# hongfz16/Garment4D

Measured on AMD Instinct MI355X. Metric: point-cloud frames/s (FPS+ball_query+SA-MLP+LBS), B=8 N=8192, higher is better.
Workload: dtype f32

## Files before the change

garment4d_amd/_lib.py:

```python
import ctypes
import os
import re
import sys

_HERE = os.path.dirname(os.path.abspath(__file__))
LIB_PATH = os.environ.get("G4D_LIB_PATH") or os.path.join(_HERE, "lib", "libg4d_hip.so")
HEADER_PATH = os.path.join(os.path.dirname(_HERE), "include", "g4d.h")

RENDER_LIB_PATH = os.path.join(_HERE, "lib", "libg4d_render.so")
RENDER_HEADER_PATH = os.path.join(os.path.dirname(_HERE), "include", "g4d_render.h")
SCAN_LIB_PATH = os.path.join(_HERE, "lib", "libg4d_scan.so")
SCAN_HEADER_PATH = os.path.join(os.path.dirname(_HERE), "include", "g4d_scan.h")
FIT_LIB_PATH = os.path.join(_HERE, "lib", "libg4d_fit.so")
FIT_HEADER_PATH = os.path.join(os.path.dirname(_HERE), "include", "g4d_fit.h")
SMPL_LIB_PATH = os.path.join(_HERE, "lib", "libg4d_smpl.so")
SMPL_HEADER_PATH = os.path.join(os.path.dirname(_HERE), "include", "g4d_smpl.h")
SKIN_LIB_PATH = os.path.join(_HERE, "lib", "libg4d_skin.so")
SKIN_HEADER_PATH = os.path.join(os.path.dirname(_HERE), "include", "g4d_skin.h")
DEPTH_LIB_PATH = os.path.join(_HERE, "lib", "libg4d_depth.so")
DEPTH_HEADER_PATH = os.path.join(os.path.dirname(_HERE), "include", "g4d_depth.h")

SETS_HEADER_PATH = os.path.join(os.path.dirname(_HERE), "include", "g4d_sets.h")

_lib = None
_header = None
_more = {}


class G4DError(RuntimeError):
    pass


_SCALARS = {"int": ctypes.c_int, "float": ctypes.c_float, "long long": ctypes.c_longlong, "size_t": ctypes.c_size_t, "unsigned": ctypes.c_uint}


def _ctype(decl, where, named=True):
    base, star, rest = decl.partition("*")
    words = [w for w in base.split() if w != "const"]
    if named and not star:
        words.pop()
    base = " ".join(words)
    if star:
        return ctypes.c_char_p if base == "char" and "*" not in rest else ctypes.c_void_p
    if base == "g4d_stream_t":
        return ctypes.c_void_p
    if base not in _SCALARS:
        raise G4DError(f"include/g4d.h: {where}: no ctypes type known for `{' '.join(decl.split())}`")
    return _SCALARS[base]


def parse_header(text):
    text = re.sub(r"/\*.*?\*/", " ", text, flags=re.S)
    consts = {n: int(v, 0) for n, v in re.findall(r"^[ \t]*#[ \t]*define[ \t]+(G4D_\w+)[ \t]+(-?(?:0[xX][0-9a-fA-F]+|\d+))[ \t]*$", text, flags=re.M)}
    text = re.sub(r"^[ \t]*#.*$", "", text, flags=re.M)
    for body in re.findall(r"\benum\s+\w+\s*\{(.*?)\}", text, flags=re.S):
        consts.update((n, int(v, 0)) for n, v in re.findall(r"(G4D_\w+)\s*=\s*(-?\w+)", body))
    fields = []
    struct = re.search(r"\bstruct\s+g4d_mlp_args\s*\{(.*?)\}", text, flags=re.S)
    for decl in filter(str.strip, struct.group(1).split(";") if struct else ()):
        first, *more = decl.split(",")
        base = first.partition("*")[0] if "*" in first else first.rsplit(None, 1)[0]
        for piece in [first] + [base + " " + p for p in more]:
            fields.append((re.findall(r"\w+", piece)[-1], _ctype(piece, "g4d_mlp_args")))
    protos = {}
    for stmt in re.split(r"[;{}]", text):
        if "(" not in stmt:
            continue
        m = re.fullmatch(r"\s*([\w\s*]+?)\b(g4d_\w+)\s*\(([^()]*)\)\s*", stmt)
        if not m:
            raise G4DError(f"include/g4d.h: cannot read `{' '.join(stmt.split())}` as a prototype")
        ret, name, params = m.groups()
        params = [] if params.strip() in ("void", "") else params.split(",")
        protos[name] = (_ctype(ret, name, named=False), [_ctype(p, name) for p in params])
    return protos, fields, consts


_MLP_FAMILY_LABELS = {"G4D_MLP_STACK_F32": "g4d_mlp_stack_f32", "G4D_MLP_STACK_BF16": "g4d_mlp_stack_bf16", "G4D_MLP_WAVE_F32": "g4d_mlp_wave_f32",
                      "G4D_MLP_CHAIN_F32": "g4d_mlp_chain_f32", "G4D_MLP_CHAIN_BF16": "g4d_mlp_chain_bf16", "G4D_MLP_CHAIN_BF16X3": "g4d_mlp_chain_bf16x3"}


def _bind_header():
    global _header
    try:
        with open(HEADER_PATH) as f:
            protos, fields, consts = parse_header(f.read())
    except OSError as e:
        raise G4DError(f"{HEADER_PATH} cannot be read ({e.strerror}): the ctypes binding is derived from it. There is no fallback table.")

    class MlpArgs(ctypes.Structure):
        _fields_ = fields

        def __init__(self, **kw):
            super().__init__(size=ctypes.sizeof(MlpArgs), version=consts["G4D_MLP_ARGS_VERSION"], tap_layer=-1, **kw)

    globals().update(
        PROTOTYPES=protos, SIGNATURES={n: a for n, (r, a) in protos.items()}, RESTYPES={n: r for n, (r, a) in protos.items() if r is not ctypes.c_int},
        CONSTANTS=consts, MlpArgs=MlpArgs, _MLP_FAMILY_NAMES={consts[k]: v for k, v in _MLP_FAMILY_LABELS.items()},
        **{k[4:]: v for k, v in consts.items() if k.startswith("G4D_MLP_")})
    _header = HEADER_PATH


def __getattr__(name):
    if _header is None and not name.startswith("__"):
        _bind_header()
        if name in globals():
            return globals()[name]
    raise AttributeError(f"module {__name__!r} has no attribute {name!r}")


def lib():
    global _lib
    if _lib is None:
        if not os.path.exists(LIB_PATH):
            raise G4DError(
                f"{LIB_PATH} not found: the HIP extension is not built. Run `python -c 'import "
                f"__graft_entry__ as g; g.build()'` (or `make -C garment4d_amd/csrc`). There is no fallback path.")
        if _header is None:
            _bind_header()
        import torch
        L = ctypes.CDLL(LIB_PATH)
        for name, (restype, argtypes) in PROTOTYPES.items():
            fn = getattr(L, name)
            fn.argtypes = argtypes
            fn.restype = restype
        _lib = L
    return _lib


def load_pair(header_path, lib_path):
    if lib_path not in _more:
        lib()
        if not os.path.exists(lib_path):
            raise G4DError(f"{lib_path} not found: the HIP extension is not built. Run `python -c 'import __graft_entry__ as g; g.build()'` "
                           f"(or `make -C garment4d_amd/csrc`). There is no fallback path.")
        try:
            with open(header_path) as f:
                protos, _, consts = parse_header(f.read())
        except OSError as e:
            raise G4DError(f"{header_path} cannot be read ({e.strerror}): the ctypes binding is derived from it. There is no fallback table.")
        L = ctypes.CDLL(lib_path)
        for name, (restype, argtypes) in protos.items():
            fn = getattr(L, name)
            fn.argtypes = argtypes
            fn.restype = restype
        _more[lib_path] = (L, protos, consts)
    return _more[lib_path]


def render_lib():
    return load_pair(RENDER_HEADER_PATH, RENDER_LIB_PATH)


def scan_lib():
    return load_pair(SCAN_HEADER_PATH, SCAN_LIB_PATH)


def fit_lib():
    return load_pair(FIT_HEADER_PATH, FIT_LIB_PATH)


def smpl_lib():
    return load_pair(SMPL_HEADER_PATH, SMPL_LIB_PATH)


def skin_lib():
    return load_pair(SKIN_HEADER_PATH, SKIN_LIB_PATH)


def depth_lib():
    return load_pair(DEPTH_HEADER_PATH, DEPTH_LIB_PATH)


def sets_lib():
    return load_pair(SETS_HEADER_PATH, LIB_PATH)


def _entry(name):
    L = lib()
    if name not in PROTOTYPES:
        for M, protos, _ in _more.values():
            if name in protos:
                return getattr(M, name)
    return getattr(L, name)


_TRACE = os.environ.get("G4D_TRACE_CALLS", "0") != "0"
_TIMED = None
_UNTIMED = ("g4d_tuning_set", "g4d_tuning_set_thread", "g4d_launch_group_begin")


class timed_calls:

    def __enter__(self):
        global _TIMED
        self._rec = []
        _TIMED = self._rec
        return self

    def __exit__(self, *exc):
        global _TIMED
        _TIMED = None
        return False

    def results(self):
        import torch
        torch.cuda.synchronize()
        return [(name, ints, e0.elapsed_time(e1) * 1e3) for name, ints, e0, e1 in self._rec]


def call(name, *args):
    L = lib()
    fn = _entry(name)
    timed = _TIMED is not None and args and name not in _UNTIMED
    if _TRACE or timed:
        label, shown = name, tuple(a for a in args if isinstance(a, int) and not isinstance(a, bool) and abs(a) < (1 << 31))
        if name == "g4d_mlp_run":
            blk = args[1].contents if hasattr(args[1], "contents") else MlpArgs.from_address(args[1])
            label = _MLP_FAMILY_NAMES[args[0]] if blk.unknown_grid is None else "g4d_mlp_chain_cells_bf16"
            shown = (blk.mode, blk.rows, blk.K0, blk.ldx, blk.N, blk.P, blk.S, blk.C, blk.use_xyz, blk.n, blk.m, blk.C2, blk.C1, blk.nlayers, blk.pool)
            if _TRACE:
                print("g4d call g4d_mlp_run ->", label, *shown, file=sys.stderr)
        if _TRACE:
            print("g4d call", name, *[a for a in args if isinstance(a, (int, float)) and abs(a) < (1 << 31)], file=sys.stderr)
    if timed:
        import torch
        e0, e1 = torch.cuda.Event(enable_timing=True), torch.cuda.Event(enable_timing=True)
        e0.record()
        rc = fn(*args)
        e1.record()
        _TIMED.append((label, shown, e0, e1))
    else:
        rc = fn(*args)
    if rc != 0:
        raise G4DError(f"{name} failed with status {rc}: {L.g4d_last_error().decode(errors='replace')}")
    return rc


def host_array(ctype, values):
    return ctypes.cast((ctype * len(values))(*values), ctypes.c_void_p)


def workspace(nbytes, device):
    import torch
    return torch.empty(max(int(nbytes), 16), dtype=torch.uint8, device=device)


def ver(t):
    try:
        return t._version
    except RuntimeError:
        return None


def stream_ptr():
    import torch
    return torch.cuda.current_stream().cuda_stream
```

garment4d_amd/csrc/ball_grid.hip:

```cpp
#include <cstdlib>

#include "g4d_common.h"
#include "../../include/g4d_sets.h"
#include "ball_grid_build.h"

namespace g4d {

__global__ void __launch_bounds__(kBuildThreads) ball_grid_build_kernel(int n, int cmax, int budget, float cell_req, const float *__restrict__ xyz_all,
                                                                       unsigned char *__restrict__ ws_all, size_t ws_stride) {
    ball_grid_build_body(n, cmax, budget, cell_req, xyz_all, ws_all, ws_stride, blockIdx.x);
}

struct BgArgs {
    float radius2[4];
    int nsample[4];
    int *idx[4];
};

__device__ __forceinline__ int query_cell(float v, float lo, float inv_c, int g) {
    const float u = floorf((v - lo) * inv_c);
    return (int)fminf(fmaxf(u, -2.f), (float)(g + 1));
}

template <int NS, int FM, bool SET>
__global__ void __launch_bounds__(256) ball_grid_query_kernel(int n, int m, int qpw, const BgArgs a, const float *__restrict__ new_xyz_all,
                                                             const float *__restrict__ xyz_all, const unsigned char *__restrict__ ws_all,
                                                             size_t ws_stride, int cmax) {
    __shared__ int lst[4][NS][kCap];
    const int t = threadIdx.x, lane = t & 63;
    const int wave = __builtin_amdgcn_readfirstlane(t >> 6);
    const int b = blockIdx.y;
    const unsigned char *ws = ws_all + (size_t)b * ws_stride;
    const GridHdr *hdr = reinterpret_cast<const GridHdr *>(ws);
    const int *cellstart = reinterpret_cast<const int *>(ws + kGridHdrBytes);
    const float4 *sorted = reinterpret_cast<const float4 *>(ws + kGridHdrBytes + ((((size_t)cmax + 1) * 4 + 63) & ~(size_t)63));
    const float *xyz = xyz_all + (size_t)b * n * 3;
    const float lox = hdr->lox, loy = hdr->loy, loz = hdr->loz, inv_c = hdr->inv_c;
    const int gx = hdr->gx, gy = hdr->gy, gz = hdr->gz;
    const int ry = lane % 3 - 1, rz = (lane / 3) % 3 - 1;

    for (int qi = 0; qi < qpw; ++qi) {
        const int q = (blockIdx.x * 4 + wave) * qpw + qi;
        if (q >= m) break;
        const float *qp = new_xyz_all + ((size_t)b * m + q) * 3;
        const float qx = qp[0], qy = qp[1], qz = qp[2];
        const int cx = query_cell(qx, lox, inv_c, gx), cy = query_cell(qy, loy, inv_c, gy), cz = query_cell(qz, loz, inv_c, gz);
        const int x0 = max(cx - 1, 0), x1 = min(cx + 1, gx - 1);
        const int yy = cy + ry, zz = cz + rz;
        int s = 0, e = 0;
        if (lane < 9 && x0 <= x1 && yy >= 0 && yy < gy && zz >= 0 && zz < gz) {
            const int row = (zz * gy + yy) * gx;
            s = cellstart[row + x0];
            e = cellstart[row + x1 + 1];
        }
        int cum[10], off[9];
        cum[0] = 0;
#pragma unroll
        for (int r = 0; r < 9; ++r) {
            const int rs = __builtin_amdgcn_readlane(s, r), re = __builtin_amdgcn_readlane(e, r);
            off[r] = rs - cum[r];
            cum[r + 1] = cum[r] + (re - rs);
        }
        const int total = cum[9];
        int h[NS];
#pragma unroll
        for (int sc = 0; sc < NS; ++sc) h[sc] = 0;

        for (int j0 = 0; j0 < total; j0 += 4 * 64) {
            bool all_dense = true;
#pragma unroll
            for (int sc = 0; sc < NS; ++sc) all_dense &= h[sc] > kCap;
            if (all_dense) break;
            float4 p[4];
            bool valid[4];
#pragma unroll
            for (int u = 0; u < 4; ++u) {
                const int j = j0 + u * 64 + lane;
                valid[u] = j < total;
                int o = off[0];
#pragma unroll
                for (int r = 1; r < 9; ++r) o = (j >= cum[r]) ? off[r] : o;
                p[u] = sorted[valid[u] ? j + o : 0];
            }
#pragma unroll
            for (int u = 0; u < 4; ++u) {
                if (j0 + u * 64 >= total) break;
                const float d2 = dist2<FM>(qx - p[u].x, qy - p[u].y, qz - p[u].z);
#pragma unroll
                for (int sc = 0; sc < NS; ++sc) {
                    const bool hit = valid[u] && d2 < a.radius2[sc];
                    const unsigned long long mask = __builtin_amdgcn_ballot_w64(hit);
                    if (mask != 0ull) {
                        const int slot = h[sc] + (int)__builtin_amdgcn_mbcnt_hi((unsigned)(mask >> 32), __builtin_amdgcn_mbcnt_lo((unsigned)mask, 0u));
                        if (hit && slot < kCap) lst[wave][sc][slot] = __float_as_int(p[u].w);
                        h[sc] += __builtin_popcountll(mask);
                    }
                }
            }
        }

#pragma unroll
        for (int sc = 0; sc < NS; ++sc) {
            const int ns = a.nsample[sc];
            int *out = a.idx[sc] + ((size_t)b * m + q) * ns;
            const int hs = h[sc];
            if (hs == 0) {
                for (int l = lane; l < ns; l += 64) out[l] = 0;
            } else if (hs <= kCap) {
                int *L = lst[wave][sc];
                int hacc = hs;
                if (hs > ns) {
                    int v[kCapRegs];
#pragma unroll
                    for (int e = 0; e < kCapRegs; ++e) v[e] = (e * 64 + lane < hs) ? L[e * 64 + lane] : 0x7fffffff;
                    const int ne = (hs + 63) >> 6;
                    int lo = 0, hi = n;
                    while (lo < hi) {
                        const int mid = (lo + hi) >> 1;
                        int c = 0;
#pragma unroll
                        for (int e = 0; e < kCapRegs; ++e)
                            if (e < ne) c += __builtin_popcountll(__builtin_amdgcn_ballot_w64(v[e] < mid));
                        if (c >= ns) hi = mid; else lo = mid + 1;
                    }
                    int w = 0;
#pragma unroll
                    for (int e = 0; e < kCapRegs; ++e)
                        if (e < ne) {
                            const bool keep = v[e] < lo;
                            const unsigned long long mask = __builtin_amdgcn_ballot_w64(keep);
                            const int slot = w + (int)__builtin_amdgcn_mbcnt_hi((unsigned)(mask >> 32), __builtin_amdgcn_mbcnt_lo((unsigned)mask, 0u));
                            if (keep) L[slot] = v[e];
                            w += __builtin_popcountll(mask);
                        }
                    hacc = w;
                }
                if constexpr (SET) {
                    const int first = L[0];
                    for (int l = lane; l < ns; l += 64) out[l] = l < hacc ? L[l] : first;
                    continue;
                }
                int first = 0;
                for (int i0 = 0; i0 < hacc; i0 += 64) {
                    const int i = i0 + lane;
                    const int v = i < hacc ? L[i] : 0x7fffffff;
                    int rank = 0;
#pragma unroll 4
                    for (int j = 0; j < hacc; ++j) rank += (L[j] < v) ? 1 : 0;
                    if (i < hacc && rank < ns) out[rank] = v;
                    const unsigned long long z = __builtin_amdgcn_ballot_w64(i < hacc && rank == 0);
                    if (z != 0ull) first = __builtin_amdgcn_readlane(v, __builtin_ctzll(z));
                }
                for (int l = hacc + lane; l < ns; l += 64) out[l] = first;
            } else {
                const float r2 = a.radius2[sc];
                int cnt = 0, first = 0;
                for (int base = 0; base < n && cnt < ns; base += 64) {
                    const int k = base + lane;
                    const int kc = min(k, n - 1);
                    const float d2 = dist2<FM>(qx - xyz[kc * 3 + 0], qy - xyz[kc * 3 + 1], qz - xyz[kc * 3 + 2]);
                    const bool hit = k < n && d2 < r2;
                    const unsigned long long mask = __builtin_amdgcn_ballot_w64(hit);
                    if (mask != 0ull) {
                        if (cnt == 0) first = base + __builtin_ctzll(mask);
                        const int slot = cnt + (int)__builtin_amdgcn_mbcnt_hi((unsigned)(mask >> 32), __builtin_amdgcn_mbcnt_lo((unsigned)mask, 0u));
                        if (hit && slot < ns) out[slot] = k;
                        cnt += __builtin_popcountll(mask);
                    }
                }
                for (int l = cnt + lane; l < ns; l += 64) out[l] = first;
            }
        }
    }
}

__device__ __forceinline__ void nn3_insert_lex(float d, int k, float &b1, float &b2, float &b3, int &i1, int &i2, int &i3) {
    const bool lt1 = d < b1 || (d == b1 && k < i1), lt2 = d < b2 || (d == b2 && k < i2), lt3 = d < b3 || (d == b3 && k < i3);
    const float nb3 = lt2 ? b2 : (lt3 ? d : b3);
    const int ni3 = lt2 ? i2 : (lt3 ? k : i3);
    const float nb2 = lt1 ? b1 : (lt2 ? d : b2);
    const int ni2 = lt1 ? i1 : (lt2 ? k : i2);
    b1 = lt1 ? d : b1; i1 = lt1 ? k : i1;
    b2 = nb2; i2 = ni2; b3 = nb3; i3 = ni3;
}

template <int FM, bool STAGE>
__global__ void __launch_bounds__(256) three_nn_grid_kernel(int n, int m, const float *__restrict__ unknown_all,
                                                           const unsigned char *__restrict__ ws_all, size_t ws_stride, int cmax,
                                                           float *__restrict__ dist2_all, int *__restrict__ idx_all) {
    extern __shared__ __attribute__((aligned(16))) unsigned char nn_smem[];
    const int b = blockIdx.y;
    const int p = blockIdx.x * 256 + threadIdx.x;
    const unsigned char *ws = ws_all + (size_t)b * ws_stride;
    const GridHdr h = *reinterpret_cast<const GridHdr *>(ws);
    const int *cellstart = reinterpret_cast<const int *>(ws + kGridHdrBytes);
    const float4 *rec = reinterpret_cast<const float4 *>(ws + kGridHdrBytes + ((((size_t)cmax + 1) * 4 + 63) & ~(size_t)63));
    if constexpr (STAGE) {
        float4 *srec = reinterpret_cast<float4 *>(nn_smem);
        int *scell = reinterpret_cast<int *>(nn_smem + (size_t)m * 16);
        for (int k = threadIdx.x; k < m; k += 256) srec[k] = rec[k];
        for (int k = threadIdx.x; k <= h.ncells; k += 256) scell[k] = cellstart[k];
        __syncthreads();
        rec = srec;
        cellstart = scell;
    }
    const float *u = unknown_all + ((size_t)b * n + min(p, n - 1)) * 3;
    const float ux = u[0], uy = u[1], uz = u[2];
    const float INF = __builtin_inff();
    float b1 = INF, b2 = INF, b3 = INF;
    int i1 = 0, i2 = 0, i3 = 0;
    auto visit = [&](int k0, int k1) {
        int k = k0;
        for (; k + 1 < k1; k += 2) {
            const float4 r0 = rec[k], r1 = rec[k + 1];
            const float d0 = dist2<FM>(ux - r0.x, uy - r0.y, uz - r0.z);
            const float d1 = dist2<FM>(ux - r1.x, uy - r1.y, uz - r1.z);
            nn3_insert_lex(d0, __float_as_int(r0.w), b1, b2, b3, i1, i2, i3);
            nn3_insert_lex(d1, __float_as_int(r1.w), b1, b2, b3, i1, i2, i3);
        }
        if (k < k1) {
            const float4 r0 = rec[k];
            nn3_insert_lex(dist2<FM>(ux - r0.x, uy - r0.y, uz - r0.z), __float_as_int(r0.w), b1, b2, b3, i1, i2, i3);
        }
    };
    const float fx = (ux - h.lox) * h.inv_c, fy = (uy - h.loy) * h.inv_c, fz = (uz - h.loz) * h.inv_c;
    bool pending = true;
    const bool local = fx > -1.f && fx < (float)h.gx + 1.f && fy > -1.f && fy < (float)h.gy + 1.f && fz > -1.f && fz < (float)h.gz + 1.f;
    if (local) {
        const int cx = (int)floorf(fx), cy = (int)floorf(fy), cz = (int)floorf(fz);
        const float edge = h.inv_c > 0.f ? 1.0f / h.inv_c : INF;
        {
            const int x0 = max(cx - 1, 0), x1 = min(cx + 1, h.gx - 1);
            int rs[9], re[9];
#pragma unroll
            for (int q = 0; q < 9; ++q) {
                const int y = cy + (q % 3) - 1, z = cz + (q / 3) - 1;
                const bool ok = x0 <= x1 && y >= 0 && y < h.gy && z >= 0 && z < h.gz;
                const int row = ok ? (z * h.gy + y) * h.gx : 0;
                rs[q] = ok ? cellstart[row + x0] : 0;
                re[q] = ok ? cellstart[row + x1 + 1] : 0;
            }
#pragma unroll
            for (int q = 0; q < 9; ++q) visit(rs[q], re[q]);
            const float reach = edge * 0.99f;
            pending = !(b3 < reach * reach);
        }
        if (pending) {
            b1 = b2 = b3 = INF; i1 = i2 = i3 = 0;
            const int x0 = max(cx - 2, 0), x1 = min(cx + 2, h.gx - 1);
            if (x0 <= x1) {
                for (int dz = -2; dz <= 2; ++dz) {
                    const int z = cz + dz;
                    if (z < 0 || z >= h.gz) continue;
                    for (int dy = -2; dy <= 2; ++dy) {
                        const int y = cy + dy;
                        if (y < 0 || y >= h.gy) continue;
                        const int row = (z * h.gy + y) * h.gx;
                        visit(cellstart[row + x0], cellstart[row + x1 + 1]);
                    }
                }
            }
            const float reach = 2.f * edge * 0.99f;
            pending = !(b3 < reach * reach);
        }
    }
    if (pending) {
        b1 = b2 = b3 = INF; i1 = i2 = i3 = 0;
        visit(0, m);
    }
    if (p < n) {
        float *d2 = dist2_all + ((size_t)b * n + p) * 3;
        int *ix = idx_all + ((size_t)b * n + p) * 3;
        d2[0] = b1; d2[1] = b2; d2[2] = b3;
        ix[0] = i1; ix[1] = i2; ix[2] = i3;
    }
}

void grid_sorted_layout(int n, size_t *offset_bytes, size_t *stride_bytes) {
    *offset_bytes = kGridHdrBytes + ((((size_t)grid_cmax(n) + 1) * 4 + 63) & ~(size_t)63);
    *stride_bytes = grid_cloud_bytes(n);
}

int grid_build(int b, int n, float rmax, const float *xyz, void *ws, hipStream_t st, int budget) {
    const int cmax = grid_cmax(n);
    if (budget <= 0 || budget > cmax) budget = cmax;
    const size_t lds = ((size_t)cmax + 1) * 4 + 16 * 8 * 4;
    static unsigned long long attr = 0;
    if (const int rc = ensure_dynamic_lds(reinterpret_cast<const void *>(ball_grid_build_kernel), 160 * 1024 - 1024, attr, "g4d_ball_grid_build_f32"))
        return rc;
    hipLaunchKernelGGL(ball_grid_build_kernel, dim3(b), dim3(kBuildThreads), lds, st, n, cmax, budget, rmax > 0.f ? rmax * kCellSlack : 0.f, xyz,
                       reinterpret_cast<unsigned char *>(ws), grid_cloud_bytes(n));
    return check_launch("g4d_ball_grid_build_f32");
}

size_t grid_bytes_per_cloud(int n) { return grid_cloud_bytes(n); }
size_t grid_records_offset(int n) { return kGridHdrBytes + ((((size_t)grid_cmax(n) + 1) * 4 + 63) & ~(size_t)63); }

template <int NS, int FM, bool SET>
static void grid_query_launch(dim3 grid, hipStream_t st, int n, int m, int qpw, const BgArgs &a, const float *new_xyz, const float *xyz,
                              const void *ws) {
    hipLaunchKernelGGL((ball_grid_query_kernel<NS, FM, SET>), grid, dim3(256), 0, st, n, m, qpw, a, new_xyz, xyz,
                       reinterpret_cast<const unsigned char *>(ws), grid_cloud_bytes(n), grid_cmax(n));
}

template <bool SET>
static int grid_query(int b, int n, int m, int nscales, const float *radii, const int *nsamples, const float *new_xyz, const float *xyz,
                      int *const *idx, const void *ws, hipStream_t st) {
    BgArgs a = {};
    for (int s = 0; s < nscales; ++s) {
        a.radius2[s] = radii[s] * radii[s];
        a.nsample[s] = nsamples[s];
        a.idx[s] = idx[s];
    }
    const long long queries = (long long)b * m;
    int qpw = 1;
    while (qpw < 8 && queries / (qpw * 2) >= 32768) qpw <<= 1;
    static const int qpw_env = env_int("G4D_BG_QPW", 0);
    if (qpw_env > 0) qpw = qpw_env;
    dim3 grid((unsigned)((m + 4 * qpw - 1) / (4 * qpw)), (unsigned)b);
    G4D_WITH_FM(distance_contraction(), switch (nscales) {
        case 1: grid_query_launch<1, FM, SET>(grid, st, n, m, qpw, a, new_xyz, xyz, ws); break;
        case 2: grid_query_launch<2, FM, SET>(grid, st, n, m, qpw, a, new_xyz, xyz, ws); break;
        case 3: grid_query_launch<3, FM, SET>(grid, st, n, m, qpw, a, new_xyz, xyz, ws); break;
        default: grid_query_launch<4, FM, SET>(grid, st, n, m, qpw, a, new_xyz, xyz, ws); break;
    })
    return check_launch(SET ? "g4d_ball_grid_query_set_f32" : "g4d_ball_grid_query_f32");
}

template <bool SET>
static int grid_query_entry(const char *name, int b, int n, int m, int nscales, const float *radii, const int *nsamples, const float *new_xyz,
                            const float *xyz, int *const *idx, const void *grid, float grid_rmax, g4d_stream_t stream) {
    G4D_REQUIRE(b >= 0 && n >= 0 && m >= 0 && nscales >= 1 && nscales <= 4 && b <= 65535, "%s: bad sizes", name);
    G4D_REQUIRE(radii && nsamples && idx, "%s: null pointer", name);
    if (b == 0 || m == 0) return G4D_OK;
    hipStream_t st = reinterpret_cast<hipStream_t>(stream);
    for (int s = 0; s < nscales; ++s) {
        G4D_REQUIRE(nsamples[s] > 0 && idx[s], "%s: bad scale %d", name, s);
        G4D_REQUIRE(radii[s] <= grid_rmax, "%s: radius %g exceeds the radius the grid was built for (%g)", name, radii[s], grid_rmax);
        if (n == 0) {
            hipError_t e = hipMemsetAsync(idx[s], 0, sizeof(int) * (size_t)b * m * nsamples[s], st);
            if (e != hipSuccess) return (int)e;
        }
    }
    if (n == 0) return G4D_OK;
    G4D_REQUIRE(new_xyz && xyz && grid, "%s: null pointer", name);
    return grid_query<SET>(b, n, m, nscales, radii, nsamples, new_xyz, xyz, idx, grid, st);
}

}

extern "C" size_t g4d_ball_grid_bytes(int b, int n) {
    if (b <= 0 || n <= 0) return 0;
    return (size_t)b * g4d::grid_cloud_bytes(n);
}

extern "C" int g4d_ball_grid_build_f32(int b, int n, float rmax, const float *xyz, void *grid, g4d_stream_t stream) {
    using namespace g4d;
    G4D_REQUIRE(b >= 0 && n >= 0 && b <= 65535, "g4d_ball_grid_build_f32: bad sizes (b=%d n=%d)", b, n);
    if (b == 0 || n == 0) return G4D_OK;
    G4D_REQUIRE(xyz && grid, "g4d_ball_grid_build_f32: null pointer");
    G4D_REQUIRE(rmax > 0.f && rmax < __builtin_inff(), "g4d_ball_grid_build_f32: rmax must be a positive finite radius");
    return grid_build(b, n, rmax, xyz, grid, reinterpret_cast<hipStream_t>(stream));
}

extern "C" int g4d_ball_grid_query_f32(int b, int n, int m, int nscales, const float *radii, const int *nsamples, const float *new_xyz,
                                       const float *xyz, int *const *idx, const void *grid, float grid_rmax, g4d_stream_t stream) {
    return g4d::grid_query_entry<false>("g4d_ball_grid_query_f32", b, n, m, nscales, radii, nsamples, new_xyz, xyz, idx, grid, grid_rmax, stream);
}

extern "C" int g4d_ball_grid_query_set_f32(int b, int n, int m, int nscales, const float *radii, const int *nsamples, const float *new_xyz,
                                           const float *xyz, int *const *idx, const void *grid, float grid_rmax, g4d_stream_t stream) {
    return g4d::grid_query_entry<true>("g4d_ball_grid_query_set_f32", b, n, m, nscales, radii, nsamples, new_xyz, xyz, idx, grid, grid_rmax, stream);
}

extern "C" int g4d_ball_query_grid_f32(int b, int n, int m, int nscales, const float *radii, const int *nsamples, const float *new_xyz,
                                       const float *xyz, int *const *idx, void *grid, g4d_stream_t stream) {
    using namespace g4d;
    G4D_REQUIRE(nscales >= 1 && nscales <= 4 && radii, "g4d_ball_query_grid_f32: bad scales");
    float rmax = radii[0];
    for (int s = 1; s < nscales; ++s) rmax = radii[s] > rmax ? radii[s] : rmax;
    if (b > 0 && n > 0 && m > 0) {
        const int rc = g4d_ball_grid_build_f32(b, n, rmax, xyz, grid, stream);
        if (rc != G4D_OK) return rc;
    }
    return g4d_ball_grid_query_f32(b, n, m, nscales, radii, nsamples, new_xyz, xyz, idx, grid, rmax, stream);
}

extern "C" int g4d_three_nn_grid_f32(int b, int n, int m, const float *unknown, const float *known, float *dist2, int *idx, void *grid,
                                     g4d_stream_t stream) {
    using namespace g4d;
    G4D_REQUIRE(b >= 0 && n >= 0 && m >= 0 && b <= 65535, "g4d_three_nn_grid_f32: bad sizes (b=%d n=%d m=%d)", b, n, m);
    if ((long long)b * n == 0) return G4D_OK;
    G4D_REQUIRE(unknown && dist2 && idx, "g4d_three_nn_grid_f32: null pointer");
    if (m == 0) return g4d_three_nn_f32(b, n, m, unknown, known, dist2, idx, stream);
    G4D_REQUIRE(known && grid, "g4d_three_nn_grid_f32: null pointer (grid scratch = g4d_ball_grid_bytes(b, m))");
    hipStream_t st = reinterpret_cast<hipStream_t>(stream);
    static const int per_cell = [] { const char *e = getenv("G4D_NN_PER_CELL"); return e && atoi(e) > 0 ? atoi(e) : 1; }();
    if (const int rc = grid_build(b, m, 0.f, known, grid, st, m / per_cell > 8 ? m / per_cell : 8)) return rc;
    dim3 g((unsigned)((n + 255) / 256), (unsigned)b);
    const unsigned char *wsb = reinterpret_cast<const unsigned char *>(grid);
    if (m <= 2048) {
        const size_t lds = (size_t)m * 16 + ((size_t)grid_cmax(m) + 1) * 4;
        G4D_WITH_FM(distance_contraction(), hipLaunchKernelGGL((three_nn_grid_kernel<FM, true>), g, dim3(256), lds, st, n, m, unknown, wsb,
                                                              grid_cloud_bytes(m), grid_cmax(m), dist2, idx))
    } else {
        G4D_WITH_FM(distance_contraction(), hipLaunchKernelGGL((three_nn_grid_kernel<FM, false>), g, dim3(256), 0, st, n, m, unknown, wsb,
                                                              grid_cloud_bytes(m), grid_cmax(m), dist2, idx))
    }
    return check_launch("g4d_three_nn_grid_f32");
}
```

garment4d_amd/csrc/fps.hip:

```cpp
#include "g4d_common.h"

namespace g4d {

template <int U>
__device__ __host__ constexpr int brev_small(int v) {
    int r = 0;
    for (int bit = 1, rb = U >> 1; bit < U; bit <<= 1, rb >>= 1)
        if (v & bit) r |= rb;
    return r;
}

struct FpsCand {
    float val;
    unsigned rank;
    int k;
    int pad;
};

__device__ __forceinline__ void wave_argmax(float best, int k, int bs, int log2bs, float &wval, int &wk, unsigned &wrank) {
    wval = wave_max_f32(best);
    const unsigned long long hit = __builtin_amdgcn_ballot_w64(best == wval);
    int lane;
    if (__builtin_popcountll(hit) == 1) {
        lane = __builtin_ctzll(hit);
        wk = __builtin_amdgcn_readlane(k, lane);
        wrank = fps_rank(wk, bs, log2bs);
    } else {
        const unsigned r = (best == wval) ? fps_rank(k, bs, log2bs) : 0xffffffffu;
        wrank = wave_min_u32(r);
        lane = __builtin_ctzll(__builtin_amdgcn_ballot_w64(r == wrank));
        wk = __builtin_amdgcn_readlane(k, lane);
    }
}

template <int W, int U, int Q, int FM>
__global__ void __launch_bounds__(64 * W) fps_reg_kernel(int n, int m, int bs, int log2bs, const float *__restrict__ xyz_all,
                                                        float *__restrict__ temp_all, int *__restrict__ idx_all, float *__restrict__ nx_all) {
    constexpr int T = 64 * W, P = U * Q;
    extern __shared__ __attribute__((aligned(16))) unsigned char smem_raw[];
    float *sx = reinterpret_cast<float *>(smem_raw + 2 * 16 * 16);
    float *sy = sx + n;
    float *sz = sy + n;
    int *spick = reinterpret_cast<int *>(sz + n);

    const int t = threadIdx.x;
    const float *xyz = xyz_all + (size_t)blockIdx.x * n * 3;
    float *temp = temp_all + (size_t)blockIdx.x * n;
    int *idx = idx_all + (size_t)blockIdx.x * m;
    float *nx = nx_all ? nx_all + (size_t)blockIdx.x * m * 3 : nullptr;

    float px[P], py[P], pz[P], md[P];
#pragma unroll
    for (int i = 0; i < P; ++i) {
        const int k = t + brev_small<U>(i / Q) * T + (i % Q) * bs;
        const bool ok = k < n;
        px[i] = ok ? xyz[k * 3 + 0] : 0.f;
        py[i] = ok ? xyz[k * 3 + 1] : 0.f;
        pz[i] = ok ? xyz[k * 3 + 2] : 0.f;
        md[i] = ok ? (temp_all ? temp[k] : 1e10f) : -2.f;
        if (ok) { sx[k] = px[i]; sy[k] = py[i]; sz[k] = pz[i]; }
    }
    if (t == 0) spick[0] = 0;
    __syncthreads();

    float x1 = sx[0], y1 = sy[0], z1 = sz[0];
    const int wave = t >> 6;
    for (int j = 1; j < m; ++j) {
        float best = -1.f;
        int bslot = 0;
#pragma unroll
        for (int i = 0; i < P; ++i) {
            const float dx = px[i] - x1, dy = py[i] - y1, dz = pz[i] - z1;
            const float d = dist2<FM>(dx, dy, dz);
            const float d2 = bare_min_f32(d, md[i]);
            md[i] = d2;
            const bool gt = d2 > best;
            bslot = gt ? i : bslot;
            best = gt ? d2 : best;
        }
        int k;
        if constexpr (P == 1) k = t;
        else k = t + brev_small<U>(bslot / Q) * T + (bslot % Q) * bs;
        float wval; int wk; unsigned wrank;
        wave_argmax(best, k, bs, log2bs, wval, wk, wrank);
        int old;
        if constexpr (W == 1) {
            old = wk;
        } else {
            unsigned long long *buf = reinterpret_cast<unsigned long long *>(smem_raw) + (j & 1) * 16;
            if ((t & 63) == 0)
                buf[wave] = ((unsigned long long)__float_as_uint(fmaxf(wval, 0.f)) << 32) | (unsigned)(~wrank);
            __syncthreads();
            const unsigned long long key = row_max_u64<W>(buf[t & (W - 1)]);
            const unsigned rank = ~(unsigned)__builtin_amdgcn_readlane((int)(unsigned)key, W - 1);
            const unsigned c = log2bs ? (__builtin_bitreverse32(rank >> 16) >> (32 - log2bs)) : 0u;
            old = (int)(((rank & 0xffffu) << log2bs) | c);
        }
        x1 = sx[old]; y1 = sy[old]; z1 = sz[old];
        if (t == 0) spick[j] = old;
    }
    if constexpr (W > 1) __syncthreads();
    for (int j = t; j < m; j += T) {
        const int k = spick[j];
        idx[j] = k;
        if (nx) { nx[j * 3 + 0] = sx[k]; nx[j * 3 + 1] = sy[k]; nx[j * 3 + 2] = sz[k]; }
    }
    if (temp_all) {
#pragma unroll
        for (int i = 0; i < P; ++i) {
            const int k = t + brev_small<U>(i / Q) * T + (i % Q) * bs;
            if (k < n) temp[k] = md[i];
        }
    }
}

template <int UA, int UB, int FM>
__global__ void __launch_bounds__(256) fps_reg_pair_kernel(int m2, const float *__restrict__ xyz_all, int *__restrict__ idx1_all,
                                                          float *__restrict__ nx1_all, int *__restrict__ idx2_all, float *__restrict__ nx2_all) {
    constexpr int T = 256, W = 4, nA = T * UA, bsA = nA, m1 = 64 * UB, bsB = m1;
    constexpr int log2bsA = UA == 1 ? 8 : (UA == 2 ? 9 : 10), log2bsB = UB == 1 ? 6 : (UB == 2 ? 7 : (UB == 4 ? 8 : 9));
    extern __shared__ __attribute__((aligned(16))) unsigned char smem_raw[];
    float *sx = reinterpret_cast<float *>(smem_raw + 2 * 16 * 16);
    float *sy = sx + nA;
    float *sz = sy + nA;
    int *spick = reinterpret_cast<int *>(sz + nA);
    float *bx = reinterpret_cast<float *>(spick + m1);
    float *by = bx + m1;
    float *bz = by + m1;
    int *spick2 = reinterpret_cast<int *>(bz + m1);
    const int t = threadIdx.x;
    const float *xyz = xyz_all + (size_t)blockIdx.x * nA * 3;

    {
        float px[UA], py[UA], pz[UA], md[UA];
#pragma unroll
        for (int i = 0; i < UA; ++i) {
            const int k = t + brev_small<UA>(i) * T;
            px[i] = xyz[k * 3 + 0]; py[i] = xyz[k * 3 + 1]; pz[i] = xyz[k * 3 + 2];
            md[i] = 1e10f;
            sx[k] = px[i]; sy[k] = py[i]; sz[k] = pz[i];
        }
        if (t == 0) spick[0] = 0;
        __syncthreads();
        float x1 = sx[0], y1 = sy[0], z1 = sz[0];
        const int wave = t >> 6;
        for (int j = 1; j < m1; ++j) {
            float best = -1.f;
            int bslot = 0;
#pragma unroll
            for (int i = 0; i < UA; ++i) {
                const float dx = px[i] - x1, dy = py[i] - y1, dz = pz[i] - z1;
                const float d = dist2<FM>(dx, dy, dz);
                const float d2 = bare_min_f32(d, md[i]);
                md[i] = d2;
                const bool gt = d2 > best;
                bslot = gt ? i : bslot;
                best = gt ? d2 : best;
            }
            const int k = UA == 1 ? t : t + brev_small<UA>(bslot) * T;
            float wval; int wk; unsigned wrank;
            wave_argmax(best, k, bsA, log2bsA, wval, wk, wrank);
            unsigned long long *buf = reinterpret_cast<unsigned long long *>(smem_raw) + (j & 1) * 16;
            if ((t & 63) == 0) buf[wave] = ((unsigned long long)__float_as_uint(fmaxf(wval, 0.f)) << 32) | (unsigned)(~wrank);
            __syncthreads();
            const unsigned long long key = row_max_u64<W>(buf[t & (W - 1)]);
            const unsigned rank = ~(unsigned)__builtin_amdgcn_readlane((int)(unsigned)key, W - 1);
            const unsigned c = __builtin_bitreverse32(rank >> 16) >> (32 - log2bsA);
            const int old = (int)(((rank & 0xffffu) << log2bsA) | c);
            x1 = sx[old]; y1 = sy[old]; z1 = sz[old];
            if (t == 0) spick[j] = old;
        }
        __syncthreads();
        int *idx = idx1_all + (size_t)blockIdx.x * m1;
        float *nx = nx1_all + (size_t)blockIdx.x * m1 * 3;
        for (int j = t; j < m1; j += T) {
            const int k = spick[j];
            idx[j] = k;
            const float x = sx[k], y = sy[k], z = sz[k];
            nx[j * 3 + 0] = x; nx[j * 3 + 1] = y; nx[j * 3 + 2] = z;
            bx[j] = x; by[j] = y; bz[j] = z;
        }
        __syncthreads();
    }
    if (t >= 64) return;
    {
        float px[UB], py[UB], pz[UB], md[UB];
#pragma unroll
        for (int i = 0; i < UB; ++i) {
            const int k = t + brev_small<UB>(i) * 64;
            px[i] = bx[k]; py[i] = by[k]; pz[i] = bz[k];
            md[i] = 1e10f;
        }
        if (t == 0) spick2[0] = 0;
        float x1 = bx[0], y1 = by[0], z1 = bz[0];
        for (int j = 1; j < m2; ++j) {
            float best = -1.f;
            int bslot = 0;
#pragma unroll
            for (int i = 0; i < UB; ++i) {
                const float dx = px[i] - x1, dy = py[i] - y1, dz = pz[i] - z1;
                const float d = dist2<FM>(dx, dy, dz);
                const float d2 = bare_min_f32(d, md[i]);
                md[i] = d2;
                const bool gt = d2 > best;
                bslot = gt ? i : bslot;
                best = gt ? d2 : best;
            }
            const int k = UB == 1 ? t : t + brev_small<UB>(bslot) * 64;
            float wval; int wk; unsigned wrank;
            wave_argmax(best, k, bsB, log2bsB, wval, wk, wrank);
            const int old = wk;
            x1 = bx[old]; y1 = by[old]; z1 = bz[old];
            if (t == 0) spick2[j] = old;
        }
        __builtin_amdgcn_fence(__ATOMIC_RELEASE, "wavefront");
        __builtin_amdgcn_wave_barrier();
        __builtin_amdgcn_fence(__ATOMIC_ACQUIRE, "wavefront");
        int *idx = idx2_all + (size_t)blockIdx.x * m2;
        float *nx = nx2_all + (size_t)blockIdx.x * m2 * 3;
        for (int j = t; j < m2; j += 64) {
            const int k = spick2[j];
            idx[j] = k;
            nx[j * 3 + 0] = bx[k]; nx[j * 3 + 1] = by[k]; nx[j * 3 + 2] = bz[k];
        }
    }
}

template <int FM>
__global__ void __launch_bounds__(1024) fps_generic_kernel(int n, int m, int bs, int log2bs, const float *__restrict__ xyz_all,
                                                          float *__restrict__ temp_all, int *__restrict__ idx_all, float *__restrict__ nx_all) {
    constexpr int W = 16;
    __shared__ FpsCand slots[2][W];
    const int t = threadIdx.x;
    const float *xyz = xyz_all + (size_t)blockIdx.x * n * 3;
    float *temp = temp_all + (size_t)blockIdx.x * n;
    int *idx = idx_all + (size_t)blockIdx.x * m;
    float *nx = nx_all ? nx_all + (size_t)blockIdx.x * m * 3 : nullptr;
    if (t == 0) idx[0] = 0;
    int old = 0;
    const int wave = t >> 6;
    for (int j = 1; j <= m; ++j) {
        const float x1 = xyz[old * 3 + 0], y1 = xyz[old * 3 + 1], z1 = xyz[old * 3 + 2];
        if (t == 0 && nx) { nx[(j - 1) * 3 + 0] = x1; nx[(j - 1) * 3 + 1] = y1; nx[(j - 1) * 3 + 2] = z1; }
        if (j == m) break;
        float best = -1.f;
        int besti = 0;
        if (t < bs) {
            for (int k = t; k < n; k += bs) {
                const float dx = xyz[k * 3 + 0] - x1, dy = xyz[k * 3 + 1] - y1, dz = xyz[k * 3 + 2] - z1;
                const float d = dist2<FM>(dx, dy, dz);
                const float d2 = fminf(d, temp[k]);
                temp[k] = d2;
                const bool gt = d2 > best;
                besti = gt ? k : besti;
                best = gt ? d2 : best;
            }
        } else {
            best = -3.f;
        }
        float wval; int wk; unsigned wrank;
        {
            wval = wave_max_f32(best);
            const unsigned r = (best == wval) ? ((t < bs ? ((log2bs ? (__builtin_bitreverse32((unsigned)t) >> (32 - log2bs)) : 0u) << 16) : 0xffff0000u) |
                                                 (unsigned)(besti >> log2bs))
                                              : 0xffffffffu;
            wrank = wave_min_u32(r);
            const int lane = __builtin_ctzll(__builtin_amdgcn_ballot_w64(r == wrank));
            wk = __builtin_amdgcn_readlane(besti, lane);
        }
        FpsCand *buf = slots[j & 1];
        if ((t & 63) == 0) { FpsCand c; c.val = wval; c.rank = wrank; c.k = wk; c.pad = 0; buf[wave] = c; }
        __syncthreads();
        FpsCand bc = buf[0];
#pragma unroll
        for (int w = 1; w < W; ++w) {
            const FpsCand c = buf[w];
            const bool take = (c.val > bc.val) || (c.val == bc.val && c.rank < bc.rank);
            bc.val = take ? c.val : bc.val;
            bc.rank = take ? c.rank : bc.rank;
            bc.k = take ? c.k : bc.k;
        }
        old = __builtin_amdgcn_readfirstlane(bc.k);
        if (t == 0) idx[j] = old;
    }
}

static int ref_block_size(int work_size) {
    const int pow_2 = (int)(std::log((double)work_size) / std::log(2.0));
    int v = 1 << pow_2;
    if (v > 1024) v = 1024;
    if (v < 1) v = 1;
    return v;
}
static int ref_block_log2(int bs) {
    int log2bs = 0;
    while ((1 << log2bs) < bs) ++log2bs;
    return log2bs;
}

template <int W, int U, int Q, int FM>
static int launch_reg_fm(int b, int n, int m, int bs, int log2bs, const float *xyz, float *temp, int *idx, float *nx, hipStream_t s) {
    const size_t lds = 2 * 16 * 16 + (size_t)n * 12 + (size_t)m * 4;
    auto kern = fps_reg_kernel<W, U, Q, FM>;
    static unsigned long long attr_done = 0;
    if (const int rc = ensure_dynamic_lds(reinterpret_cast<const void *>(kern), 160 * 1024 - 1024, attr_done, "g4d_fps_f32")) return rc;
    hipLaunchKernelGGL(kern, dim3(b), dim3(64 * W), lds, s, n, m, bs, log2bs, xyz, temp, idx, nx);
    return check_launch("g4d_fps_f32");
}

template <int W, int U, int Q>
static int launch_reg(int b, int n, int m, int bs, int log2bs, const float *xyz, float *temp, int *idx, float *nx, hipStream_t s) {
    G4D_WITH_FM(distance_contraction(), return (launch_reg_fm<W, U, Q, FM>(b, n, m, bs, log2bs, xyz, temp, idx, nx, s)))
    return G4D_OK;
}

int fps_bucket_dispatch(int b, int n, int m, int bs, int log2bs, const float *xyz, float *temp, int *idx, float *nx, hipStream_t s);
int fps_big_dispatch(int b, int n, int m, int bs, int log2bs, const float *xyz, float *temp, int *idx, float *nx, hipStream_t s);
int fps_bucket_grid_launch(int b, int n, int m, int bs, int log2bs, const float *xyz, int *idx, float *nx, float rmax, void *grid_ws, hipStream_t s);


static int g_fps_force_w = -1;

}

static int fps_impl(int b, int n, int m, const float *xyz, float *temp, int *idx, float *nx, g4d_stream_t stream) {
    using namespace g4d;
    G4D_REQUIRE(b >= 0 && n >= 0 && m >= 0, "g4d_fps_f32: negative size (b=%d n=%d m=%d)", b, n, m);
    if (b == 0 || m == 0) return G4D_OK;
    G4D_REQUIRE(n > 0, "g4d_fps_f32: n must be > 0 when m > 0");
    G4D_REQUIRE(xyz && idx, "g4d_fps_f32: null pointer");
    hipStream_t s = reinterpret_cast<hipStream_t>(stream);
    const int bs = ref_block_size(n), log2bs = ref_block_log2(bs);
    const int q =(n + bs - 1) / bs;
    if (g_fps_force_w < 0) {
        const char *e = getenv("G4D_FPS_W");
        g_fps_force_w = e ? atoi(e) : 99;
    }
    const int force = g_fps_force_w;
    static const int use_bucket = env_int("G4D_FPS_BUCKET", 1);
    if (use_bucket && force > 16 && n > (use_bucket >= 2 ? 2048 : 4096) && n <= 8192) {
        const int rc = fps_bucket_dispatch(b, n, m, bs, log2bs, xyz, temp, idx, nx, s);
        if (rc >= 0) return rc;
    }
    static const int use_big = env_int("G4D_FPS_BIG", 1);
    const bool lds_ok = (size_t)n * 12 + (size_t)m * 4 + 512 <= 158 * 1024;
    if (use_big && force > 16 && n > 8192 && n <= 32768 && (use_big >= 2 || !(lds_ok && n <= 12800))) {
        const int rc = fps_big_dispatch(b, n, m, bs, log2bs, xyz, temp, idx, nx, s);
        if (rc >= 0) return rc;
    }
#define G4D_FPS_CASE(W, U, Q) return launch_reg<W, U, Q>(b, n, m, bs, log2bs, xyz, temp, idx, nx, s)
    if (lds_ok && force != 0 && bs >= 64) {
        const int qp = q <= 1 ? 1 : q <= 2 ? 2 : q <= 4 ? 4 : q <= 8 ? 8 : q <= 16 ? 16 : 0;
        const bool want_w1 = (force == 1) || (force > 16 && n <= 512);
        if (want_w1 && qp && (bs / 64) * qp <= 32) {
            const int u = bs / 64;
            if (u == 1 && qp == 1) G4D_FPS_CASE(1, 1, 1);
            if (u == 1 && qp == 2) G4D_FPS_CASE(1, 1, 2);
            if (u == 2 && qp == 1) G4D_FPS_CASE(1, 2, 1);
            if (u == 2 && qp == 2) G4D_FPS_CASE(1, 2, 2);
            if (u == 4 && qp == 1) G4D_FPS_CASE(1, 4, 1);
            if (u == 4 && qp == 2) G4D_FPS_CASE(1, 4, 2);
            if (u == 8 && qp == 1) G4D_FPS_CASE(1, 8, 1);
            if (u == 8 && qp == 2) G4D_FPS_CASE(1, 8, 2);
            if (u == 16 && qp == 1) G4D_FPS_CASE(1, 16, 1);
            if (u == 16 && qp == 2) G4D_FPS_CASE(1, 16, 2);
        }
        const int wsel = (force == 4 || force == 8 || force == 16) ? force : (n > 2048 ? 16 : 4);
        if (wsel == 16 && bs == 1024 && qp && qp <= 8) {
            if (qp == 1) G4D_FPS_CASE(16, 1, 1);
            if (qp == 2) G4D_FPS_CASE(16, 1, 2);
            if (qp == 4) G4D_FPS_CASE(16, 1, 4);
            if (qp == 8) G4D_FPS_CASE(16, 1, 8);
        }
        if (wsel >= 8 && bs >= 512 && qp && qp <= 8) {
            const int u = bs / 512;
            if (u == 1 && qp == 1) G4D_FPS_CASE(8, 1, 1);
            if (u == 1 && qp == 2) G4D_FPS_CASE(8, 1, 2);
            if (u == 2 && qp == 1) G4D_FPS_CASE(8, 2, 1);
            if (u == 2 && qp == 2) G4D_FPS_CASE(8, 2, 2);
            if (u == 2 && qp == 4) G4D_FPS_CASE(8, 2, 4);
            if (u == 2 && qp == 8) G4D_FPS_CASE(8, 2, 8);
        }
        if (bs >= 256 && qp) {
            const int u = bs / 256;
            if (u == 1 && qp == 1) G4D_FPS_CASE(4, 1, 1);
            if (u == 1 && qp == 2) G4D_FPS_CASE(4, 1, 2);
            if (u == 2 && qp == 1) G4D_FPS_CASE(4, 2, 1);
            if (u == 2 && qp == 2) G4D_FPS_CASE(4, 2, 2);
            if (u == 4 && qp == 1) G4D_FPS_CASE(4, 4, 1);
            if (u == 4 && qp == 2) G4D_FPS_CASE(4, 4, 2);
            if (u == 4 && qp == 4) G4D_FPS_CASE(4, 4, 4);
            if (u == 4 && qp == 8) G4D_FPS_CASE(4, 4, 8);
            if (u == 4 && qp == 16) G4D_FPS_CASE(4, 4, 16);
        }
        if (bs >= 64 && bs < 256 && qp && (bs / 64) * qp <= 32) {
            const int u = bs / 64;
            if (u == 1 && qp == 1) G4D_FPS_CASE(1, 1, 1);
            if (u == 1 && qp == 2) G4D_FPS_CASE(1, 1, 2);
            if (u == 2 && qp == 1) G4D_FPS_CASE(1, 2, 1);
            if (u == 2 && qp == 2) G4D_FPS_CASE(1, 2, 2);
        }
    }
#undef G4D_FPS_CASE
    G4D_REQUIRE(temp, "g4d_fps_f32: temp scratch (B,N) is required for this N (the scratch-free kernels cover 64 <= N <= 32768)");
    G4D_WITH_FM(distance_contraction(), hipLaunchKernelGGL(fps_generic_kernel<FM>, dim3(b), dim3(1024), 0, s, n, m, bs, log2bs, xyz, temp, idx, nx))
    return check_launch("g4d_fps_f32(generic)");
}

extern "C" int g4d_fps_f32(int b, int n, int m, const float *xyz, float *temp, int *idx, g4d_stream_t stream) {
    return fps_impl(b, n, m, xyz, temp, idx, nullptr, stream);
}

extern "C" int g4d_fps_gather_f32(int b, int n, int m, const float *xyz, float *temp, int *idx, float *new_xyz, g4d_stream_t stream) {
    G4D_REQUIRE(new_xyz || b == 0 || m == 0, "g4d_fps_gather_f32: new_xyz is NULL");
    return fps_impl(b, n, m, xyz, temp, idx, new_xyz, stream);
}

extern "C" int g4d_fps_gather_pair_supported(int n, int m1, int m2) { return n == 1024 && m1 == 256 && m2 >= 1 && m2 <= m1; }
extern "C" int g4d_fps_gather_pair_f32(int b, int n, int m1, int m2, const float *xyz, int *idx1, float *new_xyz1, int *idx2, float *new_xyz2,
                                       g4d_stream_t stream) {
    using namespace g4d;
    G4D_REQUIRE(b >= 0 && g4d_fps_gather_pair_supported(n, m1, m2), "g4d_fps_gather_pair_f32: unsupported shape (n=%d m1=%d m2=%d)", n, m1, m2);
    if (b == 0) return G4D_OK;
    G4D_REQUIRE(xyz && idx1 && new_xyz1 && idx2 && new_xyz2, "g4d_fps_gather_pair_f32: null pointer");
    const size_t lds = 2 * 16 * 16 + (size_t)n * 12 + (size_t)m1 * 16 + (size_t)m2 * 4;
    hipStream_t s = reinterpret_cast<hipStream_t>(stream);
    G4D_WITH_FM(distance_contraction(), hipLaunchKernelGGL((fps_reg_pair_kernel<4, 4, FM>), dim3(b), dim3(256), lds, s, m2, xyz, idx1, new_xyz1, idx2, new_xyz2))
    return check_launch("g4d_fps_gather_pair_f32");
}

extern "C" int g4d_ball_grid_build_f32(int b, int n, float rmax, const float *xyz, void *grid, g4d_stream_t stream);
extern "C" int g4d_fps_gather_grid_f32(int b, int n, int m, const float *xyz, int *idx, float *new_xyz, float rmax, void *grid, g4d_stream_t stream) {
    using namespace g4d;
    G4D_REQUIRE(b >= 0 && n > 0 && m > 0 && rmax > 0.f, "g4d_fps_gather_grid_f32: bad sizes");
    if (b == 0) return G4D_OK;
    G4D_REQUIRE(xyz && idx && new_xyz && grid, "g4d_fps_gather_grid_f32: null pointer");
    static const int merged = env_int("G4D_FPS_GRID_MERGED", 1);
    static const int use_bucket = env_int("G4D_FPS_BUCKET", 1);
    if (merged && use_bucket && !getenv("G4D_FPS_W") && !getenv("G4D_FPS_BUCKET_W") && !getenv("G4D_FPS_DEAL")) {
        const int bs = ref_block_size(n), log2bs = ref_block_log2(bs);
        const int rc =fps_bucket_grid_launch(b, n, m, bs, log2bs, xyz, idx, new_xyz, rmax, grid, reinterpret_cast<hipStream_t>(stream));
        if (rc >= 0) return rc;
    }
    if (const int rc = g4d_fps_gather_f32(b, n, m, xyz, nullptr, idx, new_xyz, stream)) return rc;
    return g4d_ball_grid_build_f32(b, n, rmax, xyz, grid, stream);
}
```

garment4d_amd/encoder.py:

```python
import torch
import torch.nn as nn

from . import fused
from . import pytorch_utils as pt_utils
from .tuning import current as _T
from .pointnet2_modules import PointnetFPModule, PointnetSAModule, PointnetSAModuleMSG, fused_route

CLASS_NUM = 7


class Pointnet2MSGSEG(nn.Module):
    def __init__(self, input_channels=3, use_xyz=True, bn=True, global_feat=True, num_classes=CLASS_NUM):
        super().__init__()
        self.global_feat = global_feat
        c0 = input_channels
        self.SA_modules = nn.ModuleList()
        self.SA_modules.append(PointnetSAModuleMSG(npoint=1024, radii=[0.05, 0.1], nsamples=[16, 32],
                                                   mlps=[[c0, 16, 16, 32], [c0, 32, 32, 64]], use_xyz=use_xyz, bn=bn))
        c1 = 32 + 64
        self.SA_modules.append(PointnetSAModuleMSG(npoint=256, radii=[0.1, 0.2], nsamples=[16, 32],
                                                   mlps=[[c1, 32, 32, 64], [c1, 64, 64, 128]], use_xyz=use_xyz, bn=bn))
        c2 = 64 + 128
        self.SA_modules.append(PointnetSAModuleMSG(npoint=64, radii=[0.2, 0.4], nsamples=[32, 64],
                                                   mlps=[[c2, 64, 64, 128], [c2, 128, 128, 256]], use_xyz=use_xyz, bn=bn))
        c3 = 128 + 256
        if global_feat:
            self.Middle_modules = PointnetSAModule(mlp=[c3, 256, 512], use_xyz=use_xyz, bn=bn)
        self.num_feat = 512
        self.pointwise_num_feat = 64 + 128 + 256 + 128 + 256
        self.feat_channels_list = [64, 128, 256, 128 + 256]
        self.FP_modules = nn.ModuleList()
        self.FP_modules.append(PointnetFPModule(mlp=[128 + c0, 128, 64], bn=bn))
        self.FP_modules.append(PointnetFPModule(mlp=[256 + c1, 256, 128], bn=bn))
        self.FP_modules.append(PointnetFPModule(mlp=[c3 + c2, 512, 256], bn=bn))
        self.FC_layer = nn.Sequential(pt_utils.Conv1d(64, 32, bn=True), nn.Dropout(),
                                      pt_utils.Conv1d(32, num_classes, activation=None))

    @staticmethod
    def _break_up_pc(pc):
        xyz = pc[..., 0:3].contiguous()
        features = pc[..., 3:].transpose(1, 2).contiguous() if pc.size(-1) > 3 else None
        return xyz, features

    def forward(self, pointcloud: torch.Tensor):
        stacks = [m for sa in self.SA_modules for m in sa.mlps] + [fp.mlp for fp in self.FP_modules] + [self.FC_layer]
        if self.global_feat:
            stacks += list(self.Middle_modules.mlps)
        sas = list(self.SA_modules) + ([self.Middle_modules] if self.global_feat else [])
        if _T().dropin_whole_model and fused_route(self, stacks, pointcloud) and all(sa.pool_method in ("max_pool", "avg_pool") for sa in sas):
            return self._forward_fused(pointcloud.contiguous(), channel_major=True)
        xyz, features = self._break_up_pc(pointcloud)
        l_xyz, l_features = [xyz], [features]
        for sa in self.SA_modules:
            nx, nf = sa(l_xyz[-1], l_features[-1])
            l_xyz.append(nx)
            l_features.append(nf)
        middle = self.Middle_modules(l_xyz[-1], l_features[-1])[1] if self.global_feat else None
        for i in range(-1, -(len(self.FP_modules) + 1), -1):
            l_features[i - 1] = self.FP_modules[i](l_xyz[i - 1], l_xyz[i], l_features[i - 1], l_features[i])
        sem_logits = self.FC_layer(l_features[0]).transpose(1, 2).contiguous()
        return middle, sem_logits, l_features, l_xyz

    def forward_fused(self, pointcloud: torch.Tensor, channel_major: bool = False, precision: str = "fp32"):
        assert not any(m.training for m in self.modules()) and precision in fused.PRECISIONS
        with fused.precision(precision):
            return self._forward_fused(pointcloud, channel_major)

    def _forward_fused(self, pointcloud, channel_major):
        xyz = pointcloud[..., 0:3].contiguous()
        feats = pointcloud[..., 3:].contiguous() if pointcloud.size(-1) > 3 else None
        l_xyz, l_feats = [xyz], [feats]
        grid0 = None
        if _T().overlap_sampling:
            cur = torch.cuda.current_stream(xyz.device)
            chain = fused.sampling_chain(xyz, [sa.npoint for sa in self.SA_modules])
            grid = None
            if xyz.shape[1] >= _T().grid_min_n:
                grid = fused.build_ball_grid(xyz, max(g.radius for g in self.SA_modules[0].groupers))
            for sa, (nx, ready, _sidx) in zip(self.SA_modules, chain):
                cur.wait_event(ready)
                _, nf = fused.sa_forward(sa, l_xyz[-1], l_feats[-1], new_xyz=nx, grid=grid)
                grid = None
                l_xyz.append(nx)
                l_feats.append(nf)
        else:
            SAs = list(self.SA_modules)
            pre_nx, pre_idx = {}, {}
            pre_nn = None
            if (_T().bq_multi and len(SAs) == 3 and all(sa.npoint is not None for sa in SAs) and SAs[0].npoint < _T().grid_min_n
                    and len(SAs[1].groupers) == len(SAs[2].groupers) <= 4):
                r0 = [g.radius for g in SAs[0].groupers]
                if _T().grid_min_n <= xyz.shape[1] <= 12800 and max(r0) <= 2.01 * min(r0) and xyz.shape[0] > 0:
                    pre_nx[0], grid0 = fused.fps_gather_grid(xyz, SAs[0].npoint, max(r0))
                else:
                    pre_nx[0] = fused.fps_gather(xyz, SAs[0].npoint)
                pair = fused.fps_gather_pair(pre_nx[0], SAs[1].npoint, SAs[2].npoint)
                if pair is not None:
                    pre_nx[1], pre_nx[2] = pair
                else:
                    pre_nx[1] = fused.fps_gather(pre_nx[0], SAs[1].npoint)
                    pre_nx[2] = fused.fps_gather(pre_nx[1], SAs[2].npoint)
                bq = (([g.radius for g in SAs[1].groupers], [g.nsample for g in SAs[1].groupers], pre_nx[0], pre_nx[1]),
                      ([g.radius for g in SAs[2].groupers], [g.nsample for g in SAs[2].groupers], pre_nx[1], pre_nx[2]))
                nfp_ = len(self.FP_modules)
                if _T().search_multi and _T().nn_multi and nfp_ == 3 and max(pre_nx[0].shape[1], pre_nx[1].shape[1]) < 4096:
                    pre_idx[1], pre_idx[2], nn_out = fused.search_multi(bq[0], bq[1], [(pre_nx[1], pre_nx[2]), (pre_nx[0], pre_nx[1])])
                    pre_nn = {-1: nn_out[0], -2: nn_out[1]}
                else:
                    pre_idx[1], pre_idx[2] = fused.ball_query_msg2(*bq)
            for li, sa in enumerate(self.SA_modules):
                grid = None
                radii = [g.radius for g in sa.groupers]
                if li == 0 and xyz.shape[1] >= _T().grid_min_n and sa.npoint is not None and max(radii) <= 2.01 * min(radii):
                    if grid0 is None:
                        grid0 = fused.build_ball_grid(xyz, max(radii))
                    grid = grid0
                nx, nf = fused.sa_forward(sa, l_xyz[-1], l_feats[-1], new_xyz=pre_nx.get(li), grid=grid, idxs=pre_idx.get(li))
                l_xyz.append(nx)
                l_feats.append(nf)
        middle = fused.sa_forward(self.Middle_modules, l_xyz[-1], l_feats[-1])[1] if self.global_feat else None
        nfp = len(self.FP_modules)
        inner = [i for i in range(-1, -nfp, -1) if l_xyz[i - 1].shape[1] < 4096]
        pre = {}
        if not _T().overlap_sampling and pre_nn is not None and sorted(inner) == sorted(pre_nn):
            pre = pre_nn
        elif _T().nn_multi and 2 <= len(inner) <= 4:
            pre = dict(zip(inner, fused.three_nn_multi([(l_xyz[i - 1], l_xyz[i]) for i in inner])))
        nxt_raw = None
        if nfp > 1:
            nxt_raw = fused.fp_table_layer(self.FP_modules[0], 0 if l_feats[0] is None else l_feats[0].shape[2],
                                           fused.pack_conv_stack(self.FP_modules[1].mlp)[-1].Cout, self.FC_layer)
        table0 = None
        for i in range(-1, -nfp, -1):
            r = fused.fp_forward(self.FP_modules[i], l_xyz[i - 1], l_xyz[i], l_feats[i - 1], l_feats[i], nn=pre.get(i),
                                 also_table=nxt_raw if i == -nfp + 1 else None)
            if isinstance(r, tuple):
                r, table0 = r
            l_feats[i - 1] = r
        l_feats[0], sem_logits = fused.fp_forward(self.FP_modules[0], l_xyz[0], l_xyz[1], l_feats[0], l_feats[1],
                                                  head=self.FC_layer, unknown_grid=grid0, table=table0)
        if channel_major:
            l_feats = [None if f is None else fused.channel_major_with_twin(f) for f in l_feats]
            middle = None if middle is None else fused.channel_major_with_twin(middle)
        return middle, sem_logits, l_feats, l_xyz


def seed_encoder(model: nn.Module, seed: int = 0):
    g = torch.Generator().manual_seed(seed)
    with torch.no_grad():
        for name, p in model.named_parameters():
            if p.dim() > 1:
                fan_in = p[0].numel()
                p.copy_(torch.randn(p.shape, generator=g) * (2.0 / fan_in) ** 0.5)
            elif name.endswith("bn.weight"):
                p.copy_(torch.rand(p.shape, generator=g) + 0.5)
            else:
                p.copy_(torch.randn(p.shape, generator=g) * 0.1)
        for name, b in model.named_buffers():
            if name.endswith("running_mean"):
                b.copy_(torch.randn(b.shape, generator=g) * 0.1)
            elif name.endswith("running_var"):
                b.copy_(torch.rand(b.shape, generator=g) + 0.5)
    return model
```

garment4d_amd/fused.py:

```python
import contextlib
import ctypes
import os

import torch
import torch.nn as nn

from . import _cache
from . import _lib
from . import pointnet2_utils as PU
from .tuning import current as _T

_KC = 32
_BN = 64


def _ptr(t):
    return 0 if t is None else t.data_ptr()


def _floats(values):
    return _lib.host_array(ctypes.c_float, [float(v) for v in values])


def _ints(values):
    return _lib.host_array(ctypes.c_int, [int(v) for v in values])


def _ptrs(tensors):
    return _lib.host_array(ctypes.c_void_p, [t.data_ptr() for t in tensors])


def _chk(t, dtype=torch.float32):
    assert t.is_cuda and t.dtype == dtype and t.is_contiguous(), "fused path needs contiguous HIP tensors"
    return t


class PackedLayer:
    __slots__ = ("W", "Wf", "Wf16", "Wc16", "scale", "shift", "K", "Kpad", "Cout", "relu", "_kperm", "_x3", "_raw", "_xyz_table")

    def __init__(self, weight2d, scale, shift, relu):
        cout, k = weight2d.shape
        kpad = (k + _KC - 1) // _KC * _KC
        cpad = (cout + _BN - 1) // _BN * _BN
        dev = weight2d.device
        W = torch.zeros((cpad, kpad), dtype=torch.float32, device=dev)
        W[:cout, :k] = weight2d
        sc = torch.zeros(cpad, dtype=torch.float32, device=dev)
        sh = torch.zeros(cpad, dtype=torch.float32, device=dev)
        sc[:cout] = scale
        sh[:cout] = shift
        Wf = W.view(cpad // 16, 16, kpad // 16, 4, 4).permute(0, 2, 3, 1, 4).contiguous()
        Wf16 = W.to(torch.bfloat16).view(cpad // 16, 16, kpad // 32, 4, 8).permute(0, 2, 3, 1, 4).contiguous()
        kperm = torch.tensor([[(4 * g + e) if e < 4 else (16 + 4 * g + e - 4) for e in range(8)] for g in range(4)], device=dev)
        Wc16 = W.to(torch.bfloat16).view(cpad // 16, 16, kpad // 32, 32)[..., kperm].permute(0, 2, 3, 1, 4).contiguous()
        self.W, self.Wf, self.Wf16, self.Wc16, self.scale, self.shift = W, Wf, Wf16, Wc16, sc, sh
        self.K, self.Kpad, self.Cout, self.relu = k, kpad, cout, int(relu)
        self._kperm, self._x3, self._raw, self._xyz_table = kperm, None, None, None

    def raw(self):
        if self._raw is None:
            dev = self.W.device
            self._raw = PackedLayer(self.W[:self.Cout, :self.K], torch.ones(self.Cout, device=dev), torch.zeros(self.Cout, device=dev), relu=False)
        return self._raw

    def Wc16x3(self):
        if self._x3 is None:
            W = self.W
            cpad, kpad = W.shape
            mask = torch.tensor(-65536, dtype=torch.int32, device=W.device)
            hi = (W.view(torch.int32) & mask).view(torch.float32)
            r = W - hi
            mid = (r.view(torch.int32) & mask).view(torch.float32)
            lo = r - mid
            assert torch.equal(hi + mid + lo, W) and torch.equal(lo.to(torch.bfloat16).float(), lo)
            self._x3 = tuple(p.to(torch.bfloat16).view(cpad // 16, 16, kpad // 32, 32)[..., self._kperm].permute(0, 2, 3, 1, 4).contiguous()
                             for p in (hi, mid, lo))
        return self._x3


def _fold(conv, bn):
    cout = conv.weight.shape[0]
    dev = conv.weight.device
    bias = conv.bias.detach().float() if conv.bias is not None else torch.zeros(cout, device=dev)
    if bn is None:
        return torch.ones(cout, device=dev), bias
    inv = torch.rsqrt(bn.running_var.detach().float() + bn.eps)
    g = bn.weight.detach().float() if bn.weight is not None else torch.ones(cout, device=dev)
    b = bn.bias.detach().float() if bn.bias is not None else torch.zeros(cout, device=dev)
    scale = g * inv
    shift = b + (bias - bn.running_mean.detach().float()) * scale
    return scale, shift


def _unwrap_bn(m):
    return m.bn if isinstance(m, nn.Sequential) and hasattr(m, "bn") else m


def _pack_block(block):
    conv = getattr(block, "conv", None)
    names = [n for n, _ in block.named_children()]
    act = getattr(block, "activation", None)
    if conv is None or conv.kernel_size not in ((1,), (1, 1)) or conv.stride not in ((1,), (1, 1)) or conv.padding not in ((0,), (0, 0)):
        raise NotImplementedError("fused path: 1x1 convolution blocks only; call the module's own forward() for this stack")
    if names[0] != "conv":
        raise NotImplementedError("fused path: post-activation blocks only (preact=False); call the module's own forward()")
    if "in" in names:
        raise NotImplementedError("fused path: instance norm needs per-sample statistics; call the module's own forward()")
    if not (act is None or isinstance(act, nn.ReLU)):
        raise NotImplementedError(f"fused path: ReLU or no activation only (got {type(act).__name__}); call the module's own forward()")
    bn = _unwrap_bn(block.bn) if "bn" in names else None
    scale, shift = _fold(conv, bn)
    w2 = conv.weight.detach().float().reshape(conv.weight.shape[0], -1)
    return PackedLayer(w2, scale, shift, relu=act is not None)


def _params_and_buffers(m):
    return list(m.parameters()) + list(m.buffers())


def pack_conv_stack(stack):
    return _cache.packed(stack, "packed", _params_and_buffers(stack),
                         lambda: [_pack_block(block) for block in stack.children() if not isinstance(block, nn.Dropout)])


def pack_conv_block(block):
    return _cache.packed(block, "block", _params_and_buffers(block), lambda: _pack_block(block))


def invalidate(module):
    return _cache.drop(module)


def to_point_major(x):
    _chk(x)
    B, C, N = x.shape
    out = torch.empty((B, N, C), dtype=torch.float32, device=x.device)
    _lib.call("g4d_transpose_f32", B, C, N, x.data_ptr(), out.data_ptr(), _lib.stream_ptr())
    return out


def to_channel_major(x):
    _chk(x)
    B, N, C = x.shape
    out = torch.empty((B, C, N), dtype=torch.float32, device=x.device)
    _lib.call("g4d_transpose_f32", B, N, C, x.data_ptr(), out.data_ptr(), _lib.stream_ptr())
    return out


_ver = _lib.ver


def attach_twin(cm, pm):
    v = _ver(cm)
    if v is not None:
        cm._g4d_pm = (pm, v)
    return cm


def point_major_of(cm):
    tw = getattr(cm, "_g4d_pm", None)
    if tw is not None and tw[1] == _ver(cm) and tuple(tw[0].shape) == (cm.shape[0], cm.shape[2], cm.shape[1]):
        return tw[0]
    pm = to_point_major(cm.contiguous())
    if cm.is_contiguous():
        attach_twin(cm, pm)
    return pm


def attach_grid(xyz, grid):
    v = _ver(xyz)
    if v is not None:
        xyz._g4d_grid = (grid, v)
    return grid


def grid_of(xyz):
    g = getattr(xyz, "_g4d_grid", None)
    return g[0] if g is not None and g[1] == _ver(xyz) else None


def channel_major_with_twin(pm):
    return attach_twin(to_channel_major(pm), pm)




def linear(x2d, layer, out=None, col0=0, pool=0, S=1):
    _chk(x2d)
    rows, ldx = x2d.shape
    assert ldx >= layer.K
    orow = rows // S if pool else rows
    if out is None:
        out = torch.empty((orow, layer.Cout), dtype=torch.float32, device=x2d.device)
    streams = _T().stream_gemm and not pool and rows >= 65536 and layer.Cout % 128 == 0 and layer.Kpad <= 128
    tiles = (not pool and rows >= 32768 and layer.K % 4 == 0 and ldx % 4 == 0 and layer.Cout % 128 == 0 and layer.Kpad >= 128
             and x2d.data_ptr() % 16 == 0)
    if not streams and not tiles and not pool and current_precision() == "fp32" and (layer.K % 32 != 0 or layer.Cout <= 16) and chain_fits([layer], 0, 1, 0):
        return mlp_stack(0, rows, layer.K, [layer], out, col0=col0, X=x2d, ldx=ldx)
    _lib.call("g4d_linear_f32", rows, layer.K, layer.Kpad, layer.Cout, x2d.data_ptr(), ldx, layer.W.data_ptr(),
              layer.scale.data_ptr(), layer.shift.data_ptr(), layer.relu, pool, S, out.data_ptr(), out.shape[-1], col0,
              _lib.stream_ptr())
    return out


_MAX_STACK_LDS = 150 * 1024


import contextvars

_PRECISION = contextvars.ContextVar("g4d_mlp_precision", default="fp32")
PRECISIONS = ("fp32", "bf16", "bf16x3")


def current_precision():
    return _PRECISION.get()


class precision:

    def __init__(self, mode):
        assert mode in PRECISIONS
        self.mode = mode

    def __enter__(self):
        self._tok = _PRECISION.set(self.mode)
        return self

    def __exit__(self, *exc):
        _PRECISION.reset(self._tok)
        return False




def _use_bf16(rows):
    return current_precision() == "bf16" and (rows is None or rows >= _T().bf16_min_rows)


_POOL_WINDOWS = (4, 8, 16, 32, 64)


def stack_fits(layers, pool, S, rows=None):
    if not (1 <= len(layers) <= 4) or (pool and S not in _POOL_WINDOWS):
        return False
    w = [0, 0]
    for l, L in enumerate(layers):
        w[l & 1] = max(w[l & 1], L.Kpad)
    if _use_bf16(rows):
        return 2 * 64 * (w[0] + 8 + w[1] + 8) <= _MAX_STACK_LDS
    return 4 * 64 * (w[0] + 4 + w[1] + 4) <= _MAX_STACK_LDS


_CHAIN_TILES = {(1, 1, 2), (2, 2, 4), (4, 4, 8), (8, 8, 16), (2, 2), (4, 4), (8, 8), (8, 4), (16, 8), (1,), (2,), (4,), (8,), (8, 4, 2, 1),
                (4, 2, 1), (2, 4), (4, 8), (8, 16), (16,), (16, 8, 8)}


_CHAIN_TILES_BF16 = {(1, 1, 2), (2, 2, 4), (4, 4, 8), (8, 8, 16), (2, 2), (4, 4), (8, 8), (8, 4), (16, 8), (1,), (2,), (4,), (8,), (8, 4, 2, 1)}


def chain_fits(layers, pool, S, mode, bf16=None):
    if not _T().use_chain or mode not in (0, 1, 2) or (pool and S not in _POOL_WINDOWS):
        return False
    if bf16 is None:
        bf16 = current_precision() == "bf16"
    return tuple((L.Cout + 15) // 16 for L in layers) in (_CHAIN_TILES_BF16 if bf16 else _CHAIN_TILES)


def wave_fits(layers, pool, S):
    if not _T().use_wave or not (1 <= len(layers) <= 4) or (pool and S not in _POOL_WINDOWS):
        return False
    return layers[0].Kpad == 32 and all(L.Cout <= 64 for L in layers[:-1]) and all(L.Kpad <= 64 for L in layers[1:])


def layer_arrays(layers, weight="Wf"):
    return (_ptrs([getattr(L, weight) for L in layers]), _ptrs([L.scale for L in layers]), _ptrs([L.shift for L in layers]),
            _ints([L.Kpad for L in layers]), _ints([L.Cout for L in layers]), _ints([L.relu for L in layers]))


def mlp_stack(mode, rows, K0, layers, out, col0=0, pool=0, S=1, X=None, ldx=0, group=None, interp=None, csr=None, tap=None, cells_grid=None):
    n = len(layers)
    Wp, Sc, Sh, Kp, Co, Re = layer_arrays(layers)
    gN = gP = gC = gU = 0
    gx = gn = gf = gi = 0
    if group is not None:
        gN, gP, gC, gU, xyz, new_xyz, feats, idx = group
        gx, gn, gf, gi = xyz.data_ptr(), new_xyz.data_ptr(), _ptr(feats), idx.data_ptr()
    inn = im = iC2 = iC1 = 0
    ik = isk = idd = ii = 0
    if interp is not None:
        inn, im, iC2, iC1, known, skip, dist2, nn_idx = interp
        ik, isk, idd, ii = known.data_ptr(), _ptr(skip), dist2.data_ptr(), nn_idx.data_ptr()
    cV = 0
    cr = cc = cv = 0
    if csr is not None:
        cV, rowptr, colidx, vals = csr
        cr, cc, cv = rowptr.data_ptr(), colidx.data_ptr(), vals.data_ptr()
    tl, tp, tld = (-1, 0, 0) if tap is None else (tap[0], tap[1].data_ptr(), tap[1].shape[-1])
    a = _lib.MlpArgs(mode=mode, K0=K0, rows=rows, X=_ptr(X), ldx=ldx, N=gN, P=gP, S=S, C=gC, use_xyz=gU, xyz=gx, new_xyz=gn, feats=gf, idx=gi,
                     n=inn, m=im, C2=iC2, C1=iC1, known_feats=ik, skip=isk, dist2=idd, nn_idx=ii, Vg=cV, rowptr=cr, colidx=cc, vals=cv, nlayers=n,
                     scale=Sc, shift=Sh, Kpad=Kp, Cout=Co, relu=Re, pool=pool, out=out.data_ptr(), ldo=out.shape[-1], col0=col0,
                     tap_out=tp, tap_ld=tld)
    a.tap_layer = tl
    def run(family, wptrs):
        a.W = wptrs
        a._keep = (wptrs, Sc, Sh, Kp, Co, Re)
        _lib.call("g4d_mlp_run", family, ctypes.pointer(a), _lib.stream_ptr())
        return out

    if current_precision() == "bf16" and chain_fits(layers, pool, S, mode, bf16=True):
        if mode == 2 and cells_grid is not None:
            a.unknown_grid = cells_grid.data_ptr()
        return run(_lib.MLP_CHAIN_BF16, _ptrs([L.Wc16 for L in layers]))
    if current_precision() == "bf16x3" and chain_fits(layers, pool, S, mode, bf16=True):
        return run(_lib.MLP_CHAIN_BF16X3, _ptrs([t for L in layers for t in L.Wc16x3()]))
    if _use_bf16(rows):
        return run(_lib.MLP_STACK_BF16, _ptrs([L.Wf16 for L in layers]))
    if current_precision() in ("fp32", "bf16x3") and chain_fits(layers, pool, S, mode, bf16=False):
        return run(_lib.MLP_CHAIN_F32, Wp)
    if tap is None and wave_fits(layers, pool, S):
        return run(_lib.MLP_WAVE_F32, Wp)
    return run(_lib.MLP_STACK_F32, Wp)


def _pool_rows(x2d, groups, S, out, col0, is_max):
    _lib.call("g4d_pool_rows_f32", groups, S, x2d.shape[1], x2d.data_ptr(), x2d.shape[1], out.data_ptr(), out.shape[-1],
              col0, int(is_max), _lib.stream_ptr())


def _run_stack(first_call, layers, rows, S, pool, out, col0, device):
    fused_pool = pool and S in (16, 32, 64)
    n = len(layers)
    h = None
    for i, L in enumerate(layers):
        last = i == n - 1
        if last and fused_pool:
            if i == 0:
                first_call(L, pool, out, col0)
            else:
                linear(h, L, out=out, col0=col0, pool=pool, S=S)
            return
        if last and not pool:
            if i == 0:
                first_call(L, 0, out, col0)
            else:
                linear(h, L, out=out, col0=col0)
            return
        nxt = torch.empty((rows, L.Cout), dtype=torch.float32, device=device)
        if i == 0:
            first_call(L, 0, nxt, 0)
        else:
            linear(h, L, out=nxt)
        h = nxt
    _pool_rows(h, rows // S, S, out, col0, pool == 1)




def build_ball_grid(xyz, rmax):
    _chk(xyz)
    B, N, _ = xyz.shape
    ws = _lib.workspace(_lib.lib().g4d_ball_grid_bytes(B, N), xyz.device)
    _lib.call("g4d_ball_grid_build_f32", B, N, float(rmax), xyz.data_ptr(), ws.data_ptr(), _lib.stream_ptr())
    return ws, float(rmax)


def ball_query_msg(radii, nsamples, xyz, new_xyz, coherent=False, grid=None, set_form=False):
    B, N, _ = xyz.shape
    P = new_xyz.shape[1]
    outs = [torch.empty((B, P, ns), dtype=torch.int32, device=xyz.device) for ns in nsamples]
    if grid is None:
        grid = (not coherent) and N >= _T().grid_min_n and max(radii) <= 2.01 * min(radii)
    if grid is True:
        grid = build_ball_grid(xyz, max(float(r) for r in radii)) if (B and N and P) else False
    done = 0
    while done < len(radii):
        n = min(4, len(radii) - done)
        R, NS, IP = _floats(radii[done:done + n]), _ints(nsamples[done:done + n]), _ptrs(outs[done:done + n])
        if grid:
            if set_form:
                _lib.sets_lib()
            _lib.call("g4d_ball_grid_query_set_f32" if set_form else "g4d_ball_grid_query_f32", B, N, P, n, R, NS, new_xyz.data_ptr(), xyz.data_ptr(), IP, grid[0].data_ptr(), grid[1], _lib.stream_ptr())
        elif coherent and N >= 256:
            boxes = torch.empty((B, (N + 15) // 16, 6), dtype=torch.float32, device=xyz.device)
            if _T().coherent_lanes:
                qs = _lib.workspace(_lib.lib().g4d_ball_query_lanes_qsort_bytes(B, P), xyz.device) if _T().lanes_sort else None
                _lib.call("g4d_ball_query_lanes_f32", B, N, P, n, R, NS, new_xyz.data_ptr(), xyz.data_ptr(), IP, boxes.data_ptr(), _ptr(qs), _lib.stream_ptr())
            else:
                _lib.call("g4d_ball_query_boxes_f32", B, N, P, n, R, NS, new_xyz.data_ptr(), xyz.data_ptr(), IP, boxes.data_ptr(), _lib.stream_ptr())
        else:
            _lib.call("g4d_ball_query_msg_f32", B, N, P, n, R, NS, new_xyz.data_ptr(), xyz.data_ptr(), IP, _lib.stream_ptr())
        done += n
    return outs


def _fps_needs_no_scratch(N, npoint):
    if 8192 < N <= 32768 and npoint <= N:
        if os.environ.get("G4D_FPS_BIG", "1") != "0" and "G4D_FPS_W" not in os.environ:
            return True
    return N >= 64 and N * 12 + npoint * 4 + 512 <= 158 * 1024 and N <= 12800


def fps_gather_grid(xyz, npoint, rmax):
    B, N, _ = _chk(xyz).shape
    if not _fps_needs_no_scratch(N, npoint):
        return fps_gather(xyz, npoint), build_ball_grid(xyz, rmax)
    sidx = torch.empty((B, npoint), dtype=torch.int32, device=xyz.device)
    new_xyz = torch.empty((B, npoint, 3), dtype=torch.float32, device=xyz.device)
    ws = _lib.workspace(_lib.lib().g4d_ball_grid_bytes(B, N), xyz.device)
    _lib.call("g4d_fps_gather_grid_f32", B, N, npoint, xyz.data_ptr(), sidx.data_ptr(), new_xyz.data_ptr(), float(rmax), ws.data_ptr(), _lib.stream_ptr())
    return new_xyz, (ws, float(rmax))




def fps_gather_pair(xyz, m1, m2):
    B, N, _ = _chk(xyz).shape
    if not (_T().fps_pair and B > 0 and _lib.lib().g4d_fps_gather_pair_supported(N, m1, m2)):
        return None
    dev = xyz.device
    i1, i2 = torch.empty((B, m1), dtype=torch.int32, device=dev), torch.empty((B, m2), dtype=torch.int32, device=dev)
    n1, n2 = torch.empty((B, m1, 3), dtype=torch.float32, device=dev), torch.empty((B, m2, 3), dtype=torch.float32, device=dev)
    _lib.call("g4d_fps_gather_pair_f32", B, N, m1, m2, xyz.data_ptr(), i1.data_ptr(), n1.data_ptr(), i2.data_ptr(), n2.data_ptr(), _lib.stream_ptr())
    return n1, n2




def _query_pair(q0, q1):
    assert len(q0[0]) == len(q1[0]) and q0[2].shape[0] == q1[2].shape[0]
    outs, args = [], [q0[2].shape[0], len(q0[0])]
    for radii, nsamples, xyz, new_xyz in (q0, q1):
        o = [torch.empty((xyz.shape[0], new_xyz.shape[1], k), dtype=torch.int32, device=q0[2].device) for k in nsamples]
        outs.append(o)
        args += [xyz.shape[1], new_xyz.shape[1], _floats(radii), _ints(nsamples), _chk(new_xyz).data_ptr(), _chk(xyz).data_ptr(), _ptrs(o)]
    return outs[0], outs[1], args


def ball_query_msg2(q0, q1):
    o0, o1, args = _query_pair(q0, q1)
    _lib.call("g4d_ball_query_msg2_f32", *args, _lib.stream_ptr())
    return o0, o1




def _nn_pairs(pairs, B, dev):
    outs = [(torch.empty((B, _chk(u).shape[1], 3), dtype=torch.float32, device=dev), torch.empty((B, u.shape[1], 3), dtype=torch.int32, device=dev))
            for u, k in pairs]
    return outs, [_ints([u.shape[1] for u, k in pairs]), _ints([_chk(k).shape[1] for u, k in pairs]), _ptrs([u for u, k in pairs]),
                  _ptrs([k for u, k in pairs]), _ptrs([o[0] for o in outs]), _ptrs([o[1] for o in outs])]


def search_multi(q0, q1, pairs):
    assert 1 <= len(pairs) <= 4
    o0, o1, args = _query_pair(q0, q1)
    outs, nn_args = _nn_pairs(pairs, q0[2].shape[0], q0[2].device)
    _lib.call("g4d_search_multi_f32", *args, len(pairs), *nn_args, _lib.stream_ptr())
    return o0, o1, outs


def fps_gather(xyz, npoint, sidx=None, new_xyz=None):
    B, N, _ = xyz.shape
    stream = _lib.stream_ptr()
    if sidx is None:
        sidx = torch.empty((B, npoint), dtype=torch.int32, device=xyz.device)
    if new_xyz is None:
        new_xyz = torch.empty((B, npoint, 3), dtype=torch.float32, device=xyz.device)
    reg = _fps_needs_no_scratch(N, npoint)
    temp = None if reg else torch.full((B, N), 1e10, dtype=torch.float32, device=xyz.device)
    _lib.call("g4d_fps_gather_f32", B, N, npoint, xyz.data_ptr(), _ptr(temp), sidx.data_ptr(), new_xyz.data_ptr(), stream)
    return new_xyz


_side_streams = {}


def side_stream(device=None):
    cur = torch.cuda.current_stream(device)
    key = (cur.device.index, cur.cuda_stream)
    st = _side_streams.get(key)
    if st is None:
        st = _side_streams[key] = torch.cuda.Stream(device=cur.device)
    return st


def sampling_chain(xyz, npoints):
    cur = torch.cuda.current_stream(xyz.device)
    B = xyz.shape[0]
    bufs = [(torch.empty((B, m), dtype=torch.int32, device=xyz.device), torch.empty((B, m, 3), dtype=torch.float32, device=xyz.device))
            for m in npoints]
    side = side_stream(xyz.device)
    side.wait_stream(cur)
    out = []
    with torch.cuda.stream(side):
        src = xyz
        for (sidx, nx), m in zip(bufs, npoints):
            fps_gather(src, m, sidx, nx)
            ev = torch.cuda.Event()
            ev.record(side)
            out.append((nx, ev, sidx))
            src = nx
    return out


class launch_group:

    def __enter__(self):
        _lib.call("g4d_launch_group_begin")
        self.launches = None
        return self

    def __exit__(self, et, ev, tb):
        if et is not None:
            _lib.lib().g4d_launch_group_abort()
            return False
        n = ctypes.c_int(0)
        _lib.call("g4d_launch_group_end", _lib.stream_ptr(), ctypes.addressof(n))
        self.launches = n.value
        return False






def sa_table_fits(layers, C, use_xyz, pool, S, table_rows, grouped_rows):
    if not (_T().sa_table and _T().use_chain and C > 0 and use_xyz and len(layers) >= 2 and current_precision() == "fp32" and table_rows < grouped_rows):
        return False
    L0, rest = layers[0], layers[1:]
    return bool(L0.relu and L0.Cout % 16 == 0 and L0.K == 3 + C and chain_fits(rest, pool, S, 1))


def sa_level_table(sa, packed, feats_pm, scales):
    firsts = [packed[k][0] for k in scales]

    def build():
        Wf = torch.cat([L.W[:L.Cout, 3:L.K] for L in firsts], 0).contiguous()
        cat = PackedLayer(Wf, torch.ones(Wf.shape[0], device=Wf.device), torch.zeros(Wf.shape[0], device=Wf.device), relu=False)
        return cat, [L.W[:L.Cout, :3].t().contiguous() for L in firsts], firsts

    cat, wx, _ = _cache.packed(sa, "sa_table", (), build, extra=tuple(id(L) for L in firsts))
    B, N, C = feats_pm.shape
    table = linear(feats_pm.view(B * N, C), cat)
    offs, c0 = [], 0
    for k, w in zip(scales, wx):
        offs.append((c0, w))
        c0 += packed[k][0].Cout
    return table, offs


def sa_scale_mlp(xyz, new_xyz, feats_pm, idx, layers, use_xyz, pool, out, col0, table=None, tab_ld=None):
    B, N, _ = xyz.shape
    P, S = idx.shape[1], idx.shape[2]
    C = 0 if feats_pm is None else feats_pm.shape[2]
    stream = _lib.stream_ptr()
    if table is not None:
        tab, c0, wxT = table
        L0, rest = layers[0], layers[1:]
        nws = int(_lib.lib().g4d_sa_table_ws_bytes(B * P * S, L0.Cout, S, pool)) if len(rest) == 2 else 0
        ws = _lib.workspace(nws, xyz.device) if nws > 0 else None
        _lib.call("g4d_mlp_chain_group_table_ws_f32", B * P * S, N, P, S, xyz.data_ptr(), new_xyz.data_ptr(), idx.data_ptr(),
                  tab.data_ptr() + 4 * c0, tab.shape[-1] if tab_ld is None else tab_ld, L0.Cout, wxT.data_ptr(), L0.scale.data_ptr(), L0.shift.data_ptr(), len(rest),
                  *layer_arrays(rest), pool, out.data_ptr(), out.shape[-1], col0, _ptr(ws), nws, stream)
        return

    def first(L, pl, o, c0):
        _lib.call("g4d_group_linear_f32", B, N, P, S, C, use_xyz, xyz.data_ptr(), new_xyz.data_ptr(),
                  _ptr(feats_pm), idx.data_ptr(), L.Kpad, L.Cout, L.W.data_ptr(), L.scale.data_ptr(),
                  L.shift.data_ptr(), L.relu, pl, o.data_ptr(), o.shape[-1], c0, stream)

    if (_T().use_sa_xyz and C == 0 and use_xyz and len(layers) == 3 and current_precision() == "fp32" and all(L.relu for L in layers)
            and B * N * 12 < 2 ** 32 and _lib.lib().g4d_sa_xyz_mlp3_supported(layers[0].Cout, layers[1].Cout, layers[2].Cout, S)):
        L1, L2, L3 = layers
        _lib.call("g4d_sa_xyz_mlp3_f32", B, N, P, S, xyz.data_ptr(), new_xyz.data_ptr(), idx.data_ptr(), L1.Cout, L2.Cout, L3.Cout,
                  L1.W.data_ptr(), L1.Kpad, L1.scale.data_ptr(), L1.shift.data_ptr(), L2.Wf.data_ptr(), L2.Kpad, L2.scale.data_ptr(),
                  L2.shift.data_ptr(), L3.Wf.data_ptr(), L3.Kpad, L3.scale.data_ptr(), L3.shift.data_ptr(), pool, out.data_ptr(),
                  out.shape[-1], col0, stream)
    elif (_T().sa_xyz_table and C == 0 and use_xyz and len(layers) == 3 and current_precision() == "fp32" and all(L.relu for L in layers) and pool == 1
          and layers[1].Cout == layers[0].Cout and layers[2].Cout == 2 * layers[0].Cout
          and layers[1].Kpad == layers[0].Cout and layers[2].Kpad == layers[0].Cout
          and _lib.lib().g4d_sa_table_supported(B * P * S, layers[0].Cout, S, pool)):
        L0 = layers[0]
        hit = L0._xyz_table
        if hit is None:
            with torch.no_grad():
                hit = (torch.zeros(128, dtype=torch.float32, device=xyz.device), L0.W[:L0.Cout, :3].t().contiguous())
            L0._xyz_table = hit
        sa_scale_mlp(xyz, new_xyz, None, idx, layers, use_xyz, pool, out, col0, table=(hit[0].view(1, -1), 0, hit[1]), tab_ld=0)
    elif _T().use_stack and stack_fits(layers, pool, S, rows=B * P * S):
        mlp_stack(1, B * P * S, (3 if use_xyz else 0) + C, layers, out, col0=col0, pool=pool, S=S,
                  group=(N, P, C, use_xyz, xyz, new_xyz, feats_pm, idx))
    else:
        _run_stack(first, layers, B * P * S, S, pool, out, col0, xyz.device)


def sa_forward(sa, xyz, feats_pm=None, new_xyz=None, grid=None, idxs=None):
    assert not any(m.training for m in sa.modules()), "fused path is eval-mode only (train-mode BN needs batch statistics)"
    _chk(xyz)
    B, N, _ = xyz.shape
    C = 0 if feats_pm is None else _chk(feats_pm).shape[2]
    pool = {"max_pool": 1, "avg_pool": 2}[sa.pool_method]
    packed = [pack_conv_stack(m) for m in sa.mlps]
    if feats_pm is not None and tuple(feats_pm.shape[:2]) != (B, N):
        raise RuntimeError(f"set abstraction: features of {tuple(feats_pm.shape[:2])} (batch, points) for xyz of ({B}, {N})")
    for g, layers in zip(sa.groupers, packed):
        cin = (3 if (g.use_xyz or feats_pm is None) else 0) + C
        if layers[0].K != cin:
            raise RuntimeError(f"set abstraction: {cin} input channels, but the first layer expects {layers[0].K}")
    ctot = sum(p[-1].Cout for p in packed)
    stream = _lib.stream_ptr()
    if sa.npoint is not None:
        if new_xyz is None:
            new_xyz = fps_gather(xyz, sa.npoint)
        P = new_xyz.shape[1]
        out = torch.empty((B, P, ctot), dtype=torch.float32, device=xyz.device)
        col0 = 0
        if idxs is None:
            idxs = ball_query_msg([g.radius for g in sa.groupers], [g.nsample for g in sa.groupers], xyz, new_xyz, grid=grid,
                                  set_form=pool == 1 and _T().bq_set)
        if (_T().use_sa_xyz and _T().sa_xyz_pair and C == 0 and len(packed) == 2 and current_precision() == "fp32" and B * N * 12 < 2 ** 32
                and all(int(g.use_xyz) for g in sa.groupers) and all(len(L_) == 3 and all(L.relu for L in L_) for L_ in packed)
                and [L.Cout for L in packed[0]] == [16, 16, 32] and [L.Cout for L in packed[1]] == [32, 32, 64]
                and [g.nsample for g in sa.groupers] == [16, 32]):
            args = []
            c0 = 0
            for g, L_, idx in zip(sa.groupers, packed, idxs):
                L1, L2, L3 = L_
                args += [g.nsample, idx.data_ptr(), L1.W.data_ptr(), L1.Kpad, L1.scale.data_ptr(), L1.shift.data_ptr(), L2.Wf.data_ptr(), L2.Kpad,
                         L2.scale.data_ptr(), L2.shift.data_ptr(), L3.Wf.data_ptr(), L3.Kpad, L3.scale.data_ptr(), L3.shift.data_ptr(), c0]
                c0 += L3.Cout
            _lib.call("g4d_sa_xyz_mlp3_pair_f32", B, N, P, xyz.data_ptr(), new_xyz.data_ptr(), pool, out.data_ptr(), out.shape[-1], *args, stream)
            return new_xyz, out
        tab_scales = [k for k, (g, layers) in enumerate(zip(sa.groupers, packed))
                      if sa_table_fits(layers, C, int(g.use_xyz), pool, g.nsample, B * N, B * P * g.nsample)]
        table, toffs = sa_level_table(sa, packed, feats_pm, tab_scales) if tab_scales else (None, [])
        grouped = 1 < len(packed) <= 4 and len(tab_scales) == len(packed)
        with (launch_group() if grouped else contextlib.nullcontext()):
            for k, (grouper, layers, idx) in enumerate(zip(sa.groupers, packed, idxs)):
                S = grouper.nsample
                use_xyz = int(grouper.use_xyz)
                assert use_xyz or feats_pm is not None
                tb = None
                if k in tab_scales:
                    c0, wxT = toffs[tab_scales.index(k)]
                    tb = (table, c0, wxT)
                sa_scale_mlp(xyz, new_xyz, feats_pm, idx, layers, use_xyz, pool, out, col0, table=tb)
                col0 += layers[-1].Cout
        return new_xyz, out
    out = torch.empty((B, 1, ctot), dtype=torch.float32, device=xyz.device)
    idx = torch.arange(N, dtype=torch.int32, device=xyz.device).repeat(B, 1).contiguous()
    zero_c = torch.zeros((B, 1, 3), dtype=torch.float32, device=xyz.device)
    col0 = 0
    for grouper, layers in zip(sa.groupers, packed):
        use_xyz = int(grouper.use_xyz) if feats_pm is not None else 1

        def first(L, pl, o, c0, use_xyz=use_xyz):
            _lib.call("g4d_group_linear_f32", B, N, 1, N, C, use_xyz, xyz.data_ptr(), zero_c.data_ptr(), _ptr(feats_pm),
                      idx.data_ptr(), L.Kpad, L.Cout, L.W.data_ptr(), L.scale.data_ptr(), L.shift.data_ptr(), L.relu, pl,
                      o.data_ptr(), o.shape[-1], c0, stream)

        if _T().use_stack and stack_fits(layers, pool, N, rows=B * N):
            mlp_stack(1, B * N, (3 if use_xyz else 0) + C, layers, out, col0=col0, pool=pool, S=N,
                      group=(N, 1, C, use_xyz, xyz, zero_c, feats_pm, idx))
        else:
            _run_stack(first, layers, B * N, N, pool, out, col0, xyz.device)
        col0 += layers[-1].Cout
    return None, out






_NN_PRUNE_MIN_QUERIES = 262144


def three_nn_pruned(unknown, unknown_grid, known, dist2, nn_idx, sorted_out):
    B, n = dist2.shape[0], dist2.shape[1]
    m = known.shape[1]
    nws = int(_lib.lib().g4d_three_nn_pruned_ws_bytes(B))
    ws = _lib.workspace(nws, known.device)
    _lib.call("g4d_three_nn_pruned_f32", B, n, m, _ptr(unknown), 0 if unknown_grid is None else unknown_grid[0].data_ptr(), known.data_ptr(),
              dist2.data_ptr(), nn_idx.data_ptr(), int(bool(sorted_out)), ws.data_ptr(), nws, _lib.stream_ptr())


def three_nn(unknown, known, dist2=None, nn_idx=None, grid=None, unknown_grid=None):
    B, n, _ = _chk(unknown).shape
    m = _chk(known).shape[1]
    dev = unknown.device
    if dist2 is None:
        dist2 = torch.empty((B, n, 3), dtype=torch.float32, device=dev)
    if nn_idx is None:
        nn_idx = torch.empty((B, n, 3), dtype=torch.int32, device=dev)
    if _T().nn_cells and unknown_grid is not None and grid is None and n >= 4096 and 256 <= m < _T().three_nn_grid_min_m and B > 0:
        if _T().nn_prune and _lib.lib().g4d_three_nn_pruned_supported(n, m) and B <= 65535 and B * n >= _NN_PRUNE_MIN_QUERIES:
            three_nn_pruned(unknown, unknown_grid, known, dist2, nn_idx, sorted_out=False)
            return dist2, nn_idx
        _lib.call("g4d_three_nn_cells_f32", B, n, m, unknown.data_ptr(), unknown_grid[0].data_ptr(), known.data_ptr(), dist2.data_ptr(),
                  nn_idx.data_ptr(), _lib.stream_ptr())
        return dist2, nn_idx
    if grid is None:
        grid = m >= _T().three_nn_grid_min_m
    if grid and m > 0 and B * n > 0:
        ws = _lib.workspace(_lib.lib().g4d_ball_grid_bytes(B, m), dev)
        _lib.call("g4d_three_nn_grid_f32", B, n, m, unknown.data_ptr(), known.data_ptr(), dist2.data_ptr(), nn_idx.data_ptr(), ws.data_ptr(),
                  _lib.stream_ptr())
    else:
        _lib.call("g4d_three_nn_f32", B, n, m, unknown.data_ptr(), known.data_ptr(), dist2.data_ptr(), nn_idx.data_ptr(), _lib.stream_ptr())
    return dist2, nn_idx




def three_nn_multi(pairs):
    assert 1 <= len(pairs) <= 4
    outs, args = _nn_pairs(pairs, pairs[0][0].shape[0], pairs[0][0].device)
    _lib.call("g4d_three_nn_multi_f32", pairs[0][0].shape[0], len(pairs), *args, _lib.stream_ptr())
    return outs




def _fp_split(fp, L0, C2, C1):
    def build():
        W0 = L0.W[:L0.Cout, :L0.K]
        ones, zeros = torch.ones(L0.Cout, device=W0.device), torch.zeros(L0.Cout, device=W0.device)
        La = PackedLayer(W0[:, :C2].contiguous(), ones, zeros, relu=False)
        Lb = PackedLayer(W0[:, C2:C2 + C1].contiguous(), L0.scale[:L0.Cout], L0.shift[:L0.Cout], relu=bool(L0.relu))
        return La, Lb, L0

    return _cache.packed(fp, "fp_split", (), build, extra=id(L0))[:2]


def fp_table_layer(fp, C1, C2, head):
    layers = pack_conv_stack(fp.mlp)
    if not (_T().fp_table and C1 == 0 and C2 % 16 == 0 and layers[0].relu and layers[0].Cout % 16 == 0 and current_precision() == "fp32" and _T().use_chain):
        return None
    rest = layers[1:] + (pack_conv_stack(head) if head is not None else [])
    if not rest or not _lib.lib().g4d_mlp_chain_supported(len(rest), _ints([L.Cout for L in rest])):
        return None
    return layers[0].raw()


def fp_forward(fp, unknown, known, unknow_feats_pm, known_feats_pm, head=None, unknown_grid=None, nn=None, table=None, also_table=None):
    assert not any(m.training for m in fp.modules()), "fused path is eval-mode only"
    _chk(unknown)
    _chk(known_feats_pm)
    B, n, _ = unknown.shape
    layers = pack_conv_stack(fp.mlp)
    stream = _lib.stream_ptr()
    C1 = 0 if unknow_feats_pm is None else _chk(unknow_feats_pm).shape[2]
    m_want = 1 if known is None else known.shape[1]
    if tuple(known_feats_pm.shape[:2]) != (B, m_want) or (known is not None and known.shape[0] != B):
        raise RuntimeError(f"feature propagation: known features of {tuple(known_feats_pm.shape[:2])} (batch, points) for {m_want} known points")
    if unknow_feats_pm is not None and tuple(unknow_feats_pm.shape[:2]) != (B, n):
        raise RuntimeError(f"feature propagation: skip features of {tuple(unknow_feats_pm.shape[:2])} (batch, points) for ({B}, {n})")
    if C1 + known_feats_pm.shape[2] != layers[0].K:
        raise RuntimeError(f"feature propagation: {C1} + {known_feats_pm.shape[2]} input channels, but the first layer expects {layers[0].K}")
    out = torch.empty((B, n, layers[-1].Cout), dtype=torch.float32, device=unknown.device)
    if known is None:
        x = known_feats_pm.expand(B, n, known_feats_pm.shape[2])
        x = x if unknow_feats_pm is None else torch.cat([x, unknow_feats_pm], dim=2)
        h = x.reshape(B * n, -1).contiguous()
        for i, L in enumerate(layers):
            h = linear(h, L, out=out.view(B * n, -1) if i == len(layers) - 1 else None)
        return out if head is None else (out, conv_stack_forward(head, out))
    m = known.shape[1]
    C2 = known_feats_pm.shape[2]
    cells = (_T().fp_cells and _T().fp_table and _T().nn_cells and nn is None and unknown_grid is not None and C1 == 0 and n >= 4096 and 256 <= m < _T().three_nn_grid_min_m
             and B > 0 and C2 % 16 == 0 and layers[0].relu and layers[0].Cout % 16 == 0 and current_precision() == "fp32" and _T().use_chain)
    if cells:
        rest_ = layers[1:] + (pack_conv_stack(head) if head is not None else [])
        cells = bool(rest_) and bool(_lib.lib().g4d_mlp_chain_supported(len(rest_), _ints([L.Cout for L in rest_])))
    if cells:
        dist2 = torch.empty((B, n, 3), dtype=torch.float32, device=unknown.device)
        nn_idx = torch.empty((B, n, 3), dtype=torch.int32, device=unknown.device)
        if _T().nn_prune and _lib.lib().g4d_three_nn_pruned_supported(n, m) and B <= 65535 and B * n >= _NN_PRUNE_MIN_QUERIES:
            three_nn_pruned(None, unknown_grid, known, dist2, nn_idx, sorted_out=True)
        else:
            _lib.call("g4d_three_nn_cells_sorted_f32", B, n, m, unknown_grid[0].data_ptr(), known.data_ptr(), dist2.data_ptr(), nn_idx.data_ptr(), stream)
    else:
        dist2, nn_idx = nn if nn is not None else three_nn(unknown, known, unknown_grid=unknown_grid)

    def first(L, pl, o, c0):
        _lib.call("g4d_interp_linear_f32", B, n, m, C2, C1, known_feats_pm.data_ptr(), _ptr(unknow_feats_pm),
                  dist2.data_ptr(), nn_idx.data_ptr(), L.Kpad, L.Cout, L.W.data_ptr(), L.scale.data_ptr(),
                  L.shift.data_ptr(), L.relu, o.data_ptr(), o.shape[-1], c0, stream)

    if (_T().fp_table and C1 == 0 and C2 % 16 == 0 and layers[0].relu and layers[0].Cout % 16 == 0 and current_precision() == "fp32" and _T().use_chain
            and B * m < B * n):
        rest = layers[1:] + (pack_conv_stack(head) if head is not None else [])
        if rest and _lib.lib().g4d_mlp_chain_supported(len(rest), _ints([L.Cout for L in rest])):
            L0 = layers[0]
            if table is None:
                table = linear(known_feats_pm.view(B * m, C2), L0.raw())
            assert table.shape == (B * m, L0.Cout)
            nl = len(layers)
            final = torch.empty((B, n, rest[-1].Cout), dtype=torch.float32, device=unknown.device) if head is not None else out
            tap_layer, tap_t = -1, None
            if head is not None and nl > 1:
                tap_layer, tap_t = nl - 2, out.view(B * n, -1)
            in_tap = out.view(B * n, -1) if (head is not None and nl == 1) else None
            _lib.call(*(("g4d_mlp_chain_table_cells_f32", B * n, n, m, L0.Cout, table.data_ptr(), dist2.data_ptr(), nn_idx.data_ptr(), unknown_grid[0].data_ptr())
                        if cells else ("g4d_mlp_chain_table_f32", B * n, n, m, L0.Cout, table.data_ptr(), dist2.data_ptr(), nn_idx.data_ptr())),
                      L0.scale.data_ptr(), L0.shift.data_ptr(), _ptr(in_tap), 0 if in_tap is None else in_tap.shape[-1], len(rest), *layer_arrays(rest),
                      final.view(B * n, -1).data_ptr(), final.shape[-1], 0, tap_layer, _ptr(tap_t), 0 if tap_t is None else tap_t.shape[-1], stream)
            return (out, final) if head is not None else out
    if (_T().fp_table and C1 > 0 and head is None and len(layers) >= 2 and layers[0].Cout % 16 == 0 and current_precision() == "fp32" and _T().use_chain
            and m < n and chain_fits(layers, 0, 1, 2)):
        La, Lb = _fp_split(fp, layers[0], C2, C1)
        table = linear(known_feats_pm.view(B * m, C2), La)
        rest = [Lb] + layers[1:]
        tapl, tap_t, fin = -1, None, out.view(B * n, -1)
        if also_table is not None and also_table.K == layers[-1].Cout and chain_fits(rest + [also_table], 0, 1, 2):
            rest = rest + [also_table]
            tapl, tap_t = len(rest) - 2, out.view(B * n, -1)
            fin = torch.empty((B * n, also_table.Cout), dtype=torch.float32, device=unknown.device)
        _lib.call("g4d_mlp_chain_interp_init_f32", B * n, n, m, C1, unknow_feats_pm.data_ptr(), table.data_ptr(), table.shape[-1], dist2.data_ptr(),
                  nn_idx.data_ptr(), len(rest), *layer_arrays(rest), fin.data_ptr(), fin.shape[-1], 0, tapl, _ptr(tap_t),
                  0 if tap_t is None else tap_t.shape[-1], stream)
        return (out, fin) if tap_t is not None else out
    if head is not None:
        hl = pack_conv_stack(head)
        allL = layers + hl
        if _T().use_stack and stack_fits(allL, 0, 1, rows=B * n):
            logits = torch.empty((B, n, hl[-1].Cout), dtype=torch.float32, device=unknown.device)
            mlp_stack(2, B * n, C2 + C1, allL, logits.view(B * n, -1), interp=(n, m, C2, C1, known_feats_pm, unknow_feats_pm, dist2, nn_idx),
                      tap=(len(layers) - 1, out.view(B * n, -1)), cells_grid=None if unknown_grid is None else unknown_grid[0])
            return out, logits
    if (_T().fp_gemm_bf16 and current_precision() == "bf16" and len(layers) == 2 and B * n >= _T().fp_gemm_bf16_min_rows and C2 % 8 == 0 and _T().use_stack
            and stack_fits(layers, 0, 1, rows=B * n) and not chain_fits(layers, 0, 1, 2) and all(L.Kpad % 64 == 0 and L.W.shape[0] % 128 == 0 for L in layers)
            and layers[0].W.shape[0] >= layers[1].Kpad >= layers[0].Cout):
        L0, L1 = layers
        rows = B * n
        elems = _lib.lib().g4d_frag_bf16_elems
        x16 = torch.empty(elems(rows, L0.Kpad), dtype=torch.bfloat16, device=unknown.device)
        h16 = torch.empty(elems(rows, L1.Kpad), dtype=torch.bfloat16, device=unknown.device)
        _lib.call("g4d_interp_concat_frag_bf16", B, n, m, C2, C1, known_feats_pm.data_ptr(), _ptr(unknow_feats_pm), dist2.data_ptr(), nn_idx.data_ptr(),
                  L0.Kpad, x16.data_ptr(), stream)
        _lib.call("g4d_gemm_frag_bf16", rows, L0.Kpad, x16.data_ptr(), L0.Wf16.data_ptr(), L0.scale.data_ptr(), L0.shift.data_ptr(), L0.relu, L0.Cout,
                  h16.data_ptr(), L1.Kpad, 0, 0, 0, stream)
        _lib.call("g4d_gemm_frag_bf16", rows, L1.Kpad, h16.data_ptr(), L1.Wf16.data_ptr(), L1.scale.data_ptr(), L1.shift.data_ptr(), L1.relu, L1.Cout,
                  0, 0, out.data_ptr(), out.shape[-1], 0, stream)
    elif _T().use_stack and (stack_fits(layers, 0, 1, rows=B * n) or chain_fits(layers, 0, 1, 2)):
        mlp_stack(2, B * n, C2 + C1, layers, out.view(B * n, -1), interp=(n, m, C2, C1, known_feats_pm, unknow_feats_pm, dist2, nn_idx))
    elif (layers[0].Cout > 64 and _T().fp_wide_table and C1 > 0 and C1 % 4 == 0 and m < n and current_precision() == "fp32"):
        La, Lb = _fp_split(fp, layers[0], C2, C1)
        table = linear(known_feats_pm.view(B * m, C2), La)
        h = out.view(B * n, -1) if len(layers) == 1 else torch.empty((B * n, Lb.Cout), dtype=torch.float32, device=unknown.device)
        _lib.call("g4d_linear_interp_add_f32", B * n, n, m, C1, Lb.Kpad, Lb.Cout, _chk(unknow_feats_pm).data_ptr(), C1, Lb.W.data_ptr(), table.data_ptr(),
                  table.shape[-1], dist2.data_ptr(), nn_idx.data_ptr(), Lb.scale.data_ptr(), Lb.shift.data_ptr(), Lb.relu, h.data_ptr(), h.shape[-1], 0, stream)
        for i, L in enumerate(layers[1:], 1):
            h = linear(h, L, out=out.view(B * n, -1) if i == len(layers) - 1 else None)
    elif layers[0].Cout > 64 and not _T().fp_wide_fused:
        x = torch.empty((B * n, C2 + C1), dtype=torch.float32, device=unknown.device)
        _lib.call("g4d_interp_concat_f32", B, n, m, C2, C1, known_feats_pm.data_ptr(), _ptr(unknow_feats_pm), dist2.data_ptr(),
                  nn_idx.data_ptr(), x.data_ptr(), stream)
        h = x
        for i, L in enumerate(layers):
            h = linear(h, L, out=out.view(B * n, -1) if i == len(layers) - 1 else None)
    else:
        _run_stack(first, layers, B * n, 1, 0, out.view(B * n, -1), 0, unknown.device)
    if head is not None:
        return out, conv_stack_forward(head, out)
    return out


def conv_stack_forward(stack, x_pm):
    B, N, C = x_pm.shape
    h = _chk(x_pm).view(B * N, C)
    layers = pack_conv_stack(stack)
    if _T().use_stack and stack_fits(layers, 0, 1, rows=B * N):
        out = torch.empty((B * N, layers[-1].Cout), dtype=torch.float32, device=x_pm.device)
        mlp_stack(0, B * N, C, layers, out, X=h, ldx=C)
        return out.view(B, N, -1)
    for L in layers:
        h = linear(h, L)
    return h.view(B, N, -1)



_LEGACY_SWITCHES = {'USE_WAVE': 'use_wave', 'USE_STACK': 'use_stack', 'STREAM_GEMM': 'stream_gemm', 'USE_CHAIN': 'use_chain', 'OVERLAP_SAMPLING': 'overlap_sampling', 'LANES_SORT': 'lanes_sort', 'COHERENT_LANES': 'coherent_lanes', 'GRID_MIN_N': 'grid_min_n', 'FPS_PAIR': 'fps_pair', 'BQ_MULTI': 'bq_multi', 'SEARCH_MULTI': 'search_multi', 'SA_XYZ_PAIR': 'sa_xyz_pair', 'USE_SA_XYZ': 'use_sa_xyz', 'SA_XYZ_TABLE': 'sa_xyz_table', 'SA_TABLE': 'sa_table', 'THREE_NN_GRID_MIN_M': 'three_nn_grid_min_m', 'NN_CELLS': 'nn_cells', 'NN_MULTI': 'nn_multi', 'FP_WIDE_FUSED': 'fp_wide_fused', 'FP_CELLS': 'fp_cells', 'FP_TABLE': 'fp_table', 'FP_GEMM_BF16_MIN_ROWS': 'fp_gemm_bf16_min_rows', 'FP_GEMM_BF16': 'fp_gemm_bf16', 'FP_WIDE_TABLE': 'fp_wide_table'}


def __getattr__(name):
    f = _LEGACY_SWITCHES.get(name)
    if f is None:
        raise AttributeError(f"module {__name__!r} has no attribute {name!r}")
    return getattr(_T(), f)
```

garment4d_amd/tuning.py:

```python
import contextlib
import contextvars
import dataclasses
import os
from typing import Mapping, Tuple


def _env_flag(name, default):
    return os.environ.get(name, "1" if default else "0") != "0"


def _env_int(name, default):
    return int(os.environ.get(name, str(default)))


NATIVE_KEYS = ("sa_table_persistent", "sa_table_min_rows", "sa_table_128", "sa_table_oversub", "sa_table_dedup", "fp_table_persistent", "fp_table_min_rows", "gemm_tile",
               "gemm_tile_min_rows", "gemm_tile_min_cout", "gemm_tile_min_kpad", "fp_init_persistent", "fp_init_min_rows",
               "fp_head_bf16_persistent", "fp_head_bf16_min_rows", "sa_group_bf16_persistent", "sa_group_bf16_min_rows")


@dataclasses.dataclass(frozen=True)
class Tuning:
    use_wave: bool = True
    use_stack: bool = True
    use_chain: bool = True
    stream_gemm: bool = True
    bf16_min_rows: int = 0
    overlap_sampling: bool = False
    lanes_sort: bool = False
    coherent_lanes: bool = False
    grid_min_n: int = 4096
    bq_set: bool = True
    fps_pair: bool = True
    bq_multi: bool = True
    search_multi: bool = True
    three_nn_grid_min_m: int = 4096
    nn_cells: bool = True
    nn_multi: bool = True
    nn_prune: bool = True
    sa_xyz_pair: bool = True
    use_sa_xyz: bool = True
    sa_xyz_table: bool = True
    sa_table: bool = True
    fp_wide_fused: bool = False
    fp_cells: bool = True
    fp_table: bool = True
    fp_gemm_bf16: bool = True
    fp_gemm_bf16_min_rows: int = 8192
    fp_wide_table: bool = True
    dropin_fused: bool = True
    dropin_whole_model: bool = True
    use_pe_kernel: bool = True
    gcn_fuse_stack: bool = True
    gcn_autograd: bool = False
    refine_autograd: bool = False
    mgn_autograd: bool = False
    stage1_autograd: bool = False
    mlp_autograd: bool = False
    lbs_autograd: bool = False
    garment_lbs_autograd: bool = False
    lbs_fused: bool = True
    lbs_mfma: bool = True
    lbs_one_launch: bool = True
    lbs_one_launch_max_b: int = 1 << 30
    nearest_cull: bool = True
    native: Tuple[Tuple[str, int], ...] = ()

    def replace(self, **kw) -> "Tuning":
        nat = kw.pop("native", None)
        if nat is not None:
            if isinstance(nat, Mapping):
                merged = dict(self.native)
                merged.update({str(k): int(v) for k, v in nat.items()})
                nat = tuple(sorted(merged.items()))
            else:
                nat = tuple((str(k), int(v)) for k, v in nat)
            for k, _ in nat:
                if k not in NATIVE_KEYS:
                    raise KeyError(f"unknown native tuning key '{k}' (include/g4d.h lists them)")
            kw["native"] = nat
        return dataclasses.replace(self, **kw)


def from_environment() -> Tuning:
    d = Tuning()
    return Tuning(
        use_wave=_env_flag("G4D_MLP_WAVE", d.use_wave), use_chain=_env_flag("G4D_MLP_CHAIN", d.use_chain), stream_gemm=_env_flag("G4D_GEMM_STREAM", d.stream_gemm),
        bf16_min_rows=_env_int("G4D_BF16_MIN_ROWS", d.bf16_min_rows), overlap_sampling=_env_flag("G4D_OVERLAP_SAMPLING", d.overlap_sampling),
        lanes_sort=_env_flag("G4D_BQ_LANES_SORT", d.lanes_sort), coherent_lanes=_env_flag("G4D_BQ_LANES", d.coherent_lanes),
        grid_min_n=_env_int("G4D_BQ_GRID_MIN_N", d.grid_min_n), bq_set=_env_flag("G4D_BQ_SET", d.bq_set), fps_pair=_env_flag("G4D_FPS_PAIR", d.fps_pair), bq_multi=_env_flag("G4D_BQ_MULTI", d.bq_multi),
        search_multi=_env_flag("G4D_SEARCH_MULTI", d.search_multi), three_nn_grid_min_m=_env_int("G4D_NN_GRID_MIN_M", d.three_nn_grid_min_m),
        nn_cells=_env_flag("G4D_NN_CELLS", d.nn_cells), nn_multi=_env_flag("G4D_NN_MULTI", d.nn_multi), nn_prune=_env_flag("G4D_NN_PRUNE", d.nn_prune), sa_xyz_pair=_env_flag("G4D_SA_XYZ_PAIR", d.sa_xyz_pair),
        use_sa_xyz=_env_flag("G4D_SA_XYZ", d.use_sa_xyz), sa_xyz_table=_env_flag("G4D_SA_XYZ_TABLE", d.sa_xyz_table), sa_table=_env_flag("G4D_SA_TABLE", d.sa_table),
        fp_wide_fused=_env_flag("G4D_FP_WIDE_FUSED", d.fp_wide_fused), fp_cells=_env_flag("G4D_FP_CELLS", d.fp_cells), fp_table=_env_flag("G4D_FP_TABLE", d.fp_table),
        fp_gemm_bf16=_env_flag("G4D_FP_GEMM_BF16", d.fp_gemm_bf16), fp_gemm_bf16_min_rows=_env_int("G4D_FP_GEMM_BF16_MIN_ROWS", d.fp_gemm_bf16_min_rows),
        fp_wide_table=_env_flag("G4D_FP_WIDE_TABLE", d.fp_wide_table), gcn_fuse_stack=_env_flag("G4D_GCN_FUSED", d.gcn_fuse_stack), gcn_autograd=_env_flag("G4D_GCN_AUTOGRAD", d.gcn_autograd),
        refine_autograd=_env_flag("G4D_REFINE_AUTOGRAD", d.refine_autograd), mgn_autograd=_env_flag("G4D_MGN_AUTOGRAD", d.mgn_autograd),
        stage1_autograd=_env_flag("G4D_STAGE1_AUTOGRAD", d.stage1_autograd), mlp_autograd=_env_flag("G4D_MLP_AUTOGRAD", d.mlp_autograd),
        lbs_autograd=_env_flag("G4D_LBS_AUTOGRAD", d.lbs_autograd), garment_lbs_autograd=_env_flag("G4D_GARMENT_LBS_AUTOGRAD", d.garment_lbs_autograd),
        dropin_fused=_env_flag("G4D_DROPIN_FUSED", d.dropin_fused), dropin_whole_model=_env_flag("G4D_DROPIN_WHOLE", d.dropin_whole_model), lbs_mfma=_env_flag("G4D_LBS_MFMA", d.lbs_mfma), lbs_one_launch=_env_flag("G4D_LBS_ONE", d.lbs_one_launch),
        lbs_one_launch_max_b=_env_int("G4D_LBS_ONE_MAX_B", d.lbs_one_launch_max_b), nearest_cull=_env_flag("G4D_NEAREST_CULL", d.nearest_cull))


DEFAULT = from_environment()
_CURRENT = contextvars.ContextVar("g4d_tuning", default=DEFAULT)


def current() -> Tuning:
    return _CURRENT.get()


@contextlib.contextmanager
def use(t: Tuning):
    outer = _CURRENT.get()
    token = _CURRENT.set(t)
    touched = {k for k, _ in t.native} | {k for k, _ in outer.native}
    try:
        if touched:
            _apply_native(dict(t.native), touched)
        yield t
    finally:
        _CURRENT.reset(token)
        if touched:
            _apply_native(dict(outer.native), touched)


def _apply_native(values, keys):
    from . import _lib
    for k in keys:
        if k in values:
            _lib.call("g4d_tuning_set_thread", k.encode(), int(values[k]), 1)
        else:
            _lib.call("g4d_tuning_set_thread", k.encode(), 0, 0)
```

Before: 54050.

## Fuse FPS pair sampling into the first-level ball grid query launch

The ball-query body moves into a shared header, and a new kernel is added that runs the SA0 grid ball query and the FPS pair sampling for SA1/SA2 in one launch, giving each batch an extra block for the sampling. The encoder calls this merged entry when a grid exists and falls back to the separate FPS pair kernel otherwise. The aim is to drop a kernel launch and overlap the serial FPS work with the query blocks. In exchange, the long-running FPS block may extend the tail of the launch and occupies a slot in the query grid.

```diff
diff --git a/garment4d_amd/_lib.py b/garment4d_amd/_lib.py
--- a/garment4d_amd/_lib.py
+++ b/garment4d_amd/_lib.py
@@ -21,6 +21,7 @@
 DEPTH_HEADER_PATH = os.path.join(os.path.dirname(_HERE), "include", "g4d_depth.h")
 
 SETS_HEADER_PATH = os.path.join(os.path.dirname(_HERE), "include", "g4d_sets.h")
+INDEX_HEADER_PATH = os.path.join(os.path.dirname(_HERE), "include", "g4d_index.h")
 
 _lib = None
 _header = None
@@ -127,8 +128,9 @@
     return _lib
 
 
-def load_pair(header_path, lib_path):
-    if lib_path not in _more:
+def load_pair(header_path, lib_path, key=None):
+    key = key or lib_path
+    if key not in _more:
         lib()
         if not os.path.exists(lib_path):
             raise G4DError(f"{lib_path} not found: the HIP extension is not built. Run `python -c 'import __graft_entry__ as g; g.build()'` "
@@ -143,8 +145,8 @@
             fn = getattr(L, name)
             fn.argtypes = argtypes
             fn.restype = restype
-        _more[lib_path] = (L, protos, consts)
-    return _more[lib_path]
+        _more[key] = (L, protos, consts)
+    return _more[key]
 
 
 def render_lib():
@@ -173,6 +175,10 @@
 
 def sets_lib():
     return load_pair(SETS_HEADER_PATH, LIB_PATH)
+
+
+def index_lib():
+    return load_pair(INDEX_HEADER_PATH, LIB_PATH, key=INDEX_HEADER_PATH)
 
 
 def _entry(name):
diff --git a/garment4d_amd/csrc/ball_grid.hip b/garment4d_amd/csrc/ball_grid.hip
--- a/garment4d_amd/csrc/ball_grid.hip
+++ b/garment4d_amd/csrc/ball_grid.hip
@@ -3,23 +3,13 @@
 #include "g4d_common.h"
 #include "../../include/g4d_sets.h"
 #include "ball_grid_build.h"
+#include "ball_grid_query_body.h"
 
 namespace g4d {
 
 __global__ void __launch_bounds__(kBuildThreads) ball_grid_build_kernel(int n, int cmax, int budget, float cell_req, const float *__restrict__ xyz_all,
                                                                        unsigned char *__restrict__ ws_all, size_t ws_stride) {
     ball_grid_build_body(n, cmax, budget, cell_req, xyz_all, ws_all, ws_stride, blockIdx.x);
-}
-
-struct BgArgs {
-    float radius2[4];
-    int nsample[4];
-    int *idx[4];
-};
-
-__device__ __forceinline__ int query_cell(float v, float lo, float inv_c, int g) {
-    const float u = floorf((v - lo) * inv_c);
-    return (int)fminf(fmaxf(u, -2.f), (float)(g + 1));
 }
 
 template <int NS, int FM, bool SET>
@@ -27,151 +17,7 @@
                                                              const float *__restrict__ xyz_all, const unsigned char *__restrict__ ws_all,
                                                              size_t ws_stride, int cmax) {
     __shared__ int lst[4][NS][kCap];
-    const int t = threadIdx.x, lane = t & 63;
-    const int wave = __builtin_amdgcn_readfirstlane(t >> 6);
-    const int b = blockIdx.y;
-    const unsigned char *ws = ws_all + (size_t)b * ws_stride;
-    const GridHdr *hdr = reinterpret_cast<const GridHdr *>(ws);
-    const int *cellstart = reinterpret_cast<const int *>(ws + kGridHdrBytes);
-    const float4 *sorted = reinterpret_cast<const float4 *>(ws + kGridHdrBytes + ((((size_t)cmax + 1) * 4 + 63) & ~(size_t)63));
-    const float *xyz = xyz_all + (size_t)b * n * 3;
-    const float lox = hdr->lox, loy = hdr->loy, loz = hdr->loz, inv_c = hdr->inv_c;
-    const int gx = hdr->gx, gy = hdr->gy, gz = hdr->gz;
-    const int ry = lane % 3 - 1, rz = (lane / 3) % 3 - 1;
-
-    for (int qi = 0; qi < qpw; ++qi) {
-        const int q = (blockIdx.x * 4 + wave) * qpw + qi;
-        if (q >= m) break;
-        const float *qp = new_xyz_all + ((size_t)b * m + q) * 3;
-        const float qx = qp[0], qy = qp[1], qz = qp[2];
-        const int cx = query_cell(qx, lox, inv_c, gx), cy = query_cell(qy, loy, inv_c, gy), cz = query_cell(qz, loz, inv_c, gz);
-        const int x0 = max(cx - 1, 0), x1 = min(cx + 1, gx - 1);
-        const int yy = cy + ry, zz = cz + rz;
-        int s = 0, e = 0;
-        if (lane < 9 && x0 <= x1 && yy >= 0 && yy < gy && zz >= 0 && zz < gz) {
-            const int row = (zz * gy + yy) * gx;
-            s = cellstart[row + x0];
-            e = cellstart[row + x1 + 1];
-        }
-        int cum[10], off[9];
-        cum[0] = 0;
-#pragma unroll
-        for (int r = 0; r < 9; ++r) {
-            const int rs = __builtin_amdgcn_readlane(s, r), re = __builtin_amdgcn_readlane(e, r);
-            off[r] = rs - cum[r];
-            cum[r + 1] = cum[r] + (re - rs);
-        }
-        const int total = cum[9];
-        int h[NS];
-#pragma unroll
-        for (int sc = 0; sc < NS; ++sc) h[sc] = 0;
-
-        for (int j0 = 0; j0 < total; j0 += 4 * 64) {
-            bool all_dense = true;
-#pragma unroll
-            for (int sc = 0; sc < NS; ++sc) all_dense &= h[sc] > kCap;
-            if (all_dense) break;
-            float4 p[4];
-            bool valid[4];
-#pragma unroll
-            for (int u = 0; u < 4; ++u) {
-                const int j = j0 + u * 64 + lane;
-                valid[u] = j < total;
-                int o = off[0];
-#pragma unroll
-                for (int r = 1; r < 9; ++r) o = (j >= cum[r]) ? off[r] : o;
-                p[u] = sorted[valid[u] ? j + o : 0];
-            }
-#pragma unroll
-            for (int u = 0; u < 4; ++u) {
-                if (j0 + u * 64 >= total) break;
-                const float d2 = dist2<FM>(qx - p[u].x, qy - p[u].y, qz - p[u].z);
-#pragma unroll
-                for (int sc = 0; sc < NS; ++sc) {
-                    const bool hit = valid[u] && d2 < a.radius2[sc];
-                    const unsigned long long mask = __builtin_amdgcn_ballot_w64(hit);
-                    if (mask != 0ull) {
-                        const int slot = h[sc] + (int)__builtin_amdgcn_mbcnt_hi((unsigned)(mask >> 32), __builtin_amdgcn_mbcnt_lo((unsigned)mask, 0u));
-                        if (hit && slot < kCap) lst[wave][sc][slot] = __float_as_int(p[u].w);
-                        h[sc] += __builtin_popcountll(mask);
-                    }
-                }
-            }
-        }
-
-#pragma unroll
-        for (int sc = 0; sc < NS; ++sc) {
-            const int ns = a.nsample[sc];
-            int *out = a.idx[sc] + ((size_t)b * m + q) * ns;
-            const int hs = h[sc];
-            if (hs == 0) {
-                for (int l = lane; l < ns; l += 64) out[l] = 0;
-            } else if (hs <= kCap) {
-                int *L = lst[wave][sc];
-                int hacc = hs;
-                if (hs > ns) {
-                    int v[kCapRegs];
-#pragma unroll
-                    for (int e = 0; e < kCapRegs; ++e) v[e] = (e * 64 + lane < hs) ? L[e * 64 + lane] : 0x7fffffff;
-                    const int ne = (hs + 63) >> 6;
-                    int lo = 0, hi = n;
-                    while (lo < hi) {
-                        const int mid = (lo + hi) >> 1;
-                        int c = 0;
-#pragma unroll
-                        for (int e = 0; e < kCapRegs; ++e)
-                            if (e < ne) c += __builtin_popcountll(__builtin_amdgcn_ballot_w64(v[e] < mid));
-                        if (c >= ns) hi = mid; else lo = mid + 1;
-                    }
-                    int w = 0;
-#pragma unroll
-                    for (int e = 0; e < kCapRegs; ++e)
-                        if (e < ne) {
-                            const bool keep = v[e] < lo;
-                            const unsigned long long mask = __builtin_amdgcn_ballot_w64(keep);
-                            const int slot = w + (int)__builtin_amdgcn_mbcnt_hi((unsigned)(mask >> 32), __builtin_amdgcn_mbcnt_lo((unsigned)mask, 0u));
-                            if (keep) L[slot] = v[e];
-                            w += __builtin_popcountll(mask);
-                        }
-                    hacc = w;
-                }
-                if constexpr (SET) {
-                    const int first = L[0];
-                    for (int l = lane; l < ns; l += 64) out[l] = l < hacc ? L[l] : first;
-                    continue;
-                }
-                int first = 0;
-                for (int i0 = 0; i0 < hacc; i0 += 64) {
-                    const int i = i0 + lane;
-                    const int v = i < hacc ? L[i] : 0x7fffffff;
-                    int rank = 0;
-#pragma unroll 4
-                    for (int j = 0; j < hacc; ++j) rank += (L[j] < v) ? 1 : 0;
-                    if (i < hacc && rank < ns) out[rank] = v;
-                    const unsigned long long z = __builtin_amdgcn_ballot_w64(i < hacc && rank == 0);
-                    if (z != 0ull) first = __builtin_amdgcn_readlane(v, __builtin_ctzll(z));
-                }
-                for (int l = hacc + lane; l < ns; l += 64) out[l] = first;
-            } else {
-                const float r2 = a.radius2[sc];
-                int cnt = 0, first = 0;
-                for (int base = 0; base < n && cnt < ns; base += 64) {
-                    const int k = base + lane;
-                    const int kc = min(k, n - 1);
-                    const float d2 = dist2<FM>(qx - xyz[kc * 3 + 0], qy - xyz[kc * 3 + 1], qz - xyz[kc * 3 + 2]);
-                    const bool hit = k < n && d2 < r2;
-                    const unsigned long long mask = __builtin_amdgcn_ballot_w64(hit);
-                    if (mask != 0ull) {
-                        if (cnt == 0) first = base + __builtin_ctzll(mask);
-                        const int slot = cnt + (int)__builtin_amdgcn_mbcnt_hi((unsigned)(mask >> 32), __builtin_amdgcn_mbcnt_lo((unsigned)mask, 0u));
-                        if (hit && slot < ns) out[slot] = k;
-                        cnt += __builtin_popcountll(mask);
-                    }
-                }
-                for (int l = cnt + lane; l < ns; l += 64) out[l] = first;
-            }
-        }
-    }
+    ball_grid_query_body<NS, FM, SET>(lst, n, m, qpw, a, new_xyz_all, xyz_all, ws_all, ws_stride, cmax, blockIdx.x, blockIdx.y);
 }
 
 __device__ __forceinline__ void nn3_insert_lex(float d, int k, float &b1, float &b2, float &b3, int &i1, int &i2, int &i3) {
@@ -312,11 +158,7 @@
         a.nsample[s] = nsamples[s];
         a.idx[s] = idx[s];
     }
-    const long long queries = (long long)b * m;
-    int qpw = 1;
-    while (qpw < 8 && queries / (qpw * 2) >= 32768) qpw <<= 1;
-    static const int qpw_env = env_int("G4D_BG_QPW", 0);
-    if (qpw_env > 0) qpw = qpw_env;
+    const int qpw = grid_query_qpw((long long)b * m);
     dim3 grid((unsigned)((m + 4 * qpw - 1) / (4 * qpw)), (unsigned)b);
     G4D_WITH_FM(distance_contraction(), switch (nscales) {
         case 1: grid_query_launch<1, FM, SET>(grid, st, n, m, qpw, a, new_xyz, xyz, ws); break;
diff --git a/garment4d_amd/csrc/ball_grid_query_body.h b/garment4d_amd/csrc/ball_grid_query_body.h
--- /dev/null
+++ b/garment4d_amd/csrc/ball_grid_query_body.h
@@ -0,0 +1,175 @@
+#pragma once
+#include "g4d_common.h"
+#include "ball_grid_build.h"
+
+namespace g4d {
+
+struct BgArgs {
+    float radius2[4];
+    int nsample[4];
+    int *idx[4];
+};
+
+inline int grid_query_qpw(long long queries) {
+    int qpw = 1;
+    while (qpw < 8 && queries / (qpw * 2) >= 32768) qpw <<= 1;
+    static const int qpw_env = env_int("G4D_BG_QPW", 0);
+    return qpw_env > 0 ? qpw_env : qpw;
+}
+
+__device__ __forceinline__ int query_cell(float v, float lo, float inv_c, int g) {
+    const float u = floorf((v - lo) * inv_c);
+    return (int)fminf(fmaxf(u, -2.f), (float)(g + 1));
+}
+
+template <int NS, int FM, bool SET>
+__device__ __forceinline__ void ball_grid_query_body(int (*lst)[NS][kCap], int n, int m, int qpw, const BgArgs &a, const float *__restrict__ new_xyz_all,
+                                                     const float *__restrict__ xyz_all, const unsigned char *__restrict__ ws_all, size_t ws_stride,
+                                                     int cmax, int bx, int b) {
+    const int t = threadIdx.x, lane = t & 63;
+    const int wave = __builtin_amdgcn_readfirstlane(t >> 6);
+    const unsigned char *ws = ws_all + (size_t)b * ws_stride;
+    const GridHdr *hdr = reinterpret_cast<const GridHdr *>(ws);
+    const int *cellstart = reinterpret_cast<const int *>(ws + kGridHdrBytes);
+    const float4 *sorted = reinterpret_cast<const float4 *>(ws + kGridHdrBytes + ((((size_t)cmax + 1) * 4 + 63) & ~(size_t)63));
+    const float *xyz = xyz_all + (size_t)b * n * 3;
+    const float lox = hdr->lox, loy = hdr->loy, loz = hdr->loz, inv_c = hdr->inv_c;
+    const int gx = hdr->gx, gy = hdr->gy, gz = hdr->gz;
+    const int ry = lane % 3 - 1, rz = (lane / 3) % 3 - 1;
+
+    for (int qi = 0; qi < qpw; ++qi) {
+        const int q = (bx * 4 + wave) * qpw + qi;
+        if (q >= m) break;
+        const float *qp = new_xyz_all + ((size_t)b * m + q) * 3;
+        const float qx = qp[0], qy = qp[1], qz = qp[2];
+        const int cx = query_cell(qx, lox, inv_c, gx), cy = query_cell(qy, loy, inv_c, gy), cz = query_cell(qz, loz, inv_c, gz);
+        const int x0 = max(cx - 1, 0), x1 = min(cx + 1, gx - 1);
+        const int yy = cy + ry, zz = cz + rz;
+        int s = 0, e = 0;
+        if (lane < 9 && x0 <= x1 && yy >= 0 && yy < gy && zz >= 0 && zz < gz) {
+            const int row = (zz * gy + yy) * gx;
+            s = cellstart[row + x0];
+            e = cellstart[row + x1 + 1];
+        }
+        int cum[10], off[9];
+        cum[0] = 0;
+#pragma unroll
+        for (int r = 0; r < 9; ++r) {
+            const int rs = __builtin_amdgcn_readlane(s, r), re = __builtin_amdgcn_readlane(e, r);
+            off[r] = rs - cum[r];
+            cum[r + 1] = cum[r] + (re - rs);
+        }
+        const int total = cum[9];
+        int h[NS];
+#pragma unroll
+        for (int sc = 0; sc < NS; ++sc) h[sc] = 0;
+
+        for (int j0 = 0; j0 < total; j0 += 4 * 64) {
+            bool all_dense = true;
+#pragma unroll
+            for (int sc = 0; sc < NS; ++sc) all_dense &= h[sc] > kCap;
+            if (all_dense) break;
+            float4 p[4];
+            bool valid[4];
+#pragma unroll
+            for (int u = 0; u < 4; ++u) {
+                const int j = j0 + u * 64 + lane;
+                valid[u] = j < total;
+                int o = off[0];
+#pragma unroll
+                for (int r = 1; r < 9; ++r) o = (j >= cum[r]) ? off[r] : o;
+                p[u] = sorted[valid[u] ? j + o : 0];
+            }
+#pragma unroll
+            for (int u = 0; u < 4; ++u) {
+                if (j0 + u * 64 >= total) break;
+                const float d2 = dist2<FM>(qx - p[u].x, qy - p[u].y, qz - p[u].z);
+#pragma unroll
+                for (int sc = 0; sc < NS; ++sc) {
+                    const bool hit = valid[u] && d2 < a.radius2[sc];
+                    const unsigned long long mask = __builtin_amdgcn_ballot_w64(hit);
+                    if (mask != 0ull) {
+                        const int slot = h[sc] + (int)__builtin_amdgcn_mbcnt_hi((unsigned)(mask >> 32), __builtin_amdgcn_mbcnt_lo((unsigned)mask, 0u));
+                        if (hit && slot < kCap) lst[wave][sc][slot] = __float_as_int(p[u].w);
+                        h[sc] += __builtin_popcountll(mask);
+                    }
+                }
+            }
+        }
+
+#pragma unroll
+        for (int sc = 0; sc < NS; ++sc) {
+            const int ns = a.nsample[sc];
+            int *out = a.idx[sc] + ((size_t)b * m + q) * ns;
+            const int hs = h[sc];
+            if (hs == 0) {
+                for (int l = lane; l < ns; l += 64) out[l] = 0;
+            } else if (hs <= kCap) {
+                int *L = lst[wave][sc];
+                int hacc = hs;
+                if (hs > ns) {
+                    int v[kCapRegs];
+#pragma unroll
+                    for (int e = 0; e < kCapRegs; ++e) v[e] = (e * 64 + lane < hs) ? L[e * 64 + lane] : 0x7fffffff;
+                    const int ne = (hs + 63) >> 6;
+                    int lo = 0, hi = n;
+                    while (lo < hi) {
+                        const int mid = (lo + hi) >> 1;
+                        int c = 0;
+#pragma unroll
+                        for (int e = 0; e < kCapRegs; ++e)
+                            if (e < ne) c += __builtin_popcountll(__builtin_amdgcn_ballot_w64(v[e] < mid));
+                        if (c >= ns) hi = mid; else lo = mid + 1;
+                    }
+                    int w = 0;
+#pragma unroll
+                    for (int e = 0; e < kCapRegs; ++e)
+                        if (e < ne) {
+                            const bool keep = v[e] < lo;
+                            const unsigned long long mask = __builtin_amdgcn_ballot_w64(keep);
+                            const int slot = w + (int)__builtin_amdgcn_mbcnt_hi((unsigned)(mask >> 32), __builtin_amdgcn_mbcnt_lo((unsigned)mask, 0u));
+                            if (keep) L[slot] = v[e];
+                            w += __builtin_popcountll(mask);
+                        }
+                    hacc = w;
+                }
+                if constexpr (SET) {
+                    const int first = L[0];
+                    for (int l = lane; l < ns; l += 64) out[l] = l < hacc ? L[l] : first;
+                    continue;
+                }
+                int first = 0;
+                for (int i0 = 0; i0 < hacc; i0 += 64) {
+                    const int i = i0 + lane;
+                    const int v = i < hacc ? L[i] : 0x7fffffff;
+                    int rank = 0;
+#pragma unroll 4
+                    for (int j = 0; j < hacc; ++j) rank += (L[j] < v) ? 1 : 0;
+                    if (i < hacc && rank < ns) out[rank] = v;
+                    const unsigned long long z = __builtin_amdgcn_ballot_w64(i < hacc && rank == 0);
+                    if (z != 0ull) first = __builtin_amdgcn_readlane(v, __builtin_ctzll(z));
+                }
+                for (int l = hacc + lane; l < ns; l += 64) out[l] = first;
+            } else {
+                const float r2 = a.radius2[sc];
+                int cnt = 0, first = 0;
+                for (int base = 0; base < n && cnt < ns; base += 64) {
+                    const int k = base + lane;
+                    const int kc = min(k, n - 1);
+                    const float d2 = dist2<FM>(qx - xyz[kc * 3 + 0], qy - xyz[kc * 3 + 1], qz - xyz[kc * 3 + 2]);
+                    const bool hit = k < n && d2 < r2;
+                    const unsigned long long mask = __builtin_amdgcn_ballot_w64(hit);
+                    if (mask != 0ull) {
+                        if (cnt == 0) first = base + __builtin_ctzll(mask);
+                        const int slot = cnt + (int)__builtin_amdgcn_mbcnt_hi((unsigned)(mask >> 32), __builtin_amdgcn_mbcnt_lo((unsigned)mask, 0u));
+                        if (hit && slot < ns) out[slot] = k;
+                        cnt += __builtin_popcountll(mask);
+                    }
+                }
+                for (int l = cnt + lane; l < ns; l += 64) out[l] = first;
+            }
+        }
+    }
+}
+
+}
diff --git a/garment4d_amd/csrc/fps.hip b/garment4d_amd/csrc/fps.hip
--- a/garment4d_amd/csrc/fps.hip
+++ b/garment4d_amd/csrc/fps.hip
@@ -1,14 +1,7 @@
 #include "g4d_common.h"
+#include "fps_pair_body.h"
 
 namespace g4d {
-
-template <int U>
-__device__ __host__ constexpr int brev_small(int v) {
-    int r = 0;
-    for (int bit = 1, rb = U >> 1; bit < U; bit <<= 1, rb >>= 1)
-        if (v & bit) r |= rb;
-    return r;
-}
 
 struct FpsCand {
     float val;
@@ -16,22 +9,6 @@
     int k;
     int pad;
 };
-
-__device__ __forceinline__ void wave_argmax(float best, int k, int bs, int log2bs, float &wval, int &wk, unsigned &wrank) {
-    wval = wave_max_f32(best);
-    const unsigned long long hit = __builtin_amdgcn_ballot_w64(best == wval);
-    int lane;
-    if (__builtin_popcountll(hit) == 1) {
-        lane = __builtin_ctzll(hit);
-        wk = __builtin_amdgcn_readlane(k, lane);
-        wrank = fps_rank(wk, bs, log2bs);
-    } else {
-        const unsigned r = (best == wval) ? fps_rank(k, bs, log2bs) : 0xffffffffu;
-        wrank = wave_min_u32(r);
-        lane = __builtin_ctzll(__builtin_amdgcn_ballot_w64(r == wrank));
-        wk = __builtin_amdgcn_readlane(k, lane);
-    }
-}
 
 template <int W, int U, int Q, int FM>
 __global__ void __launch_bounds__(64 * W) fps_reg_kernel(int n, int m, int bs, int log2bs, const float *__restrict__ xyz_all,
@@ -117,113 +94,8 @@
 template <int UA, int UB, int FM>
 __global__ void __launch_bounds__(256) fps_reg_pair_kernel(int m2, const float *__restrict__ xyz_all, int *__restrict__ idx1_all,
                                                           float *__restrict__ nx1_all, int *__restrict__ idx2_all, float *__restrict__ nx2_all) {
-    constexpr int T = 256, W = 4, nA = T * UA, bsA = nA, m1 = 64 * UB, bsB = m1;
-    constexpr int log2bsA = UA == 1 ? 8 : (UA == 2 ? 9 : 10), log2bsB = UB == 1 ? 6 : (UB == 2 ? 7 : (UB == 4 ? 8 : 9));
     extern __shared__ __attribute__((aligned(16))) unsigned char smem_raw[];
-    float *sx = reinterpret_cast<float *>(smem_raw + 2 * 16 * 16);
-    float *sy = sx + nA;
-    float *sz = sy + nA;
-    int *spick = reinterpret_cast<int *>(sz + nA);
-    float *bx = reinterpret_cast<float *>(spick + m1);
-    float *by = bx + m1;
-    float *bz = by + m1;
-    int *spick2 = reinterpret_cast<int *>(bz + m1);
-    const int t = threadIdx.x;
-    const float *xyz = xyz_all + (size_t)blockIdx.x * nA * 3;
-
-    {
-        float px[UA], py[UA], pz[UA], md[UA];
-#pragma unroll
-        for (int i = 0; i < UA; ++i) {
-            const int k = t + brev_small<UA>(i) * T;
-            px[i] = xyz[k * 3 + 0]; py[i] = xyz[k * 3 + 1]; pz[i] = xyz[k * 3 + 2];
-            md[i] = 1e10f;
-            sx[k] = px[i]; sy[k] = py[i]; sz[k] = pz[i];
-        }
-        if (t == 0) spick[0] = 0;
-        __syncthreads();
-        float x1 = sx[0], y1 = sy[0], z1 = sz[0];
-        const int wave = t >> 6;
-        for (int j = 1; j < m1; ++j) {
-            float best = -1.f;
-            int bslot = 0;
-#pragma unroll
-            for (int i = 0; i < UA; ++i) {
-                const float dx = px[i] - x1, dy = py[i] - y1, dz = pz[i] - z1;
-                const float d = dist2<FM>(dx, dy, dz);
-                const float d2 = bare_min_f32(d, md[i]);
-                md[i] = d2;
-                const bool gt = d2 > best;
-                bslot = gt ? i : bslot;
-                best = gt ? d2 : best;
-            }
-            const int k = UA == 1 ? t : t + brev_small<UA>(bslot) * T;
-            float wval; int wk; unsigned wrank;
-            wave_argmax(best, k, bsA, log2bsA, wval, wk, wrank);
-            unsigned long long *buf = reinterpret_cast<unsigned long long *>(smem_raw) + (j & 1) * 16;
-            if ((t & 63) == 0) buf[wave] = ((unsigned long long)__float_as_uint(fmaxf(wval, 0.f)) << 32) | (unsigned)(~wrank);
-            __syncthreads();
-            const unsigned long long key = row_max_u64<W>(buf[t & (W - 1)]);
-            const unsigned rank = ~(unsigned)__builtin_amdgcn_readlane((int)(unsigned)key, W - 1);
-            const unsigned c = __builtin_bitreverse32(rank >> 16) >> (32 - log2bsA);
-            const int old = (int)(((rank & 0xffffu) << log2bsA) | c);
-            x1 = sx[old]; y1 = sy[old]; z1 = sz[old];
-            if (t == 0) spick[j] = old;
-        }
-        __syncthreads();
-        int *idx = idx1_all + (size_t)blockIdx.x * m1;
-        float *nx = nx1_all + (size_t)blockIdx.x * m1 * 3;
-        for (int j = t; j < m1; j += T) {
-            const int k = spick[j];
-            idx[j] = k;
-            const float x = sx[k], y = sy[k], z = sz[k];
-            nx[j * 3 + 0] = x; nx[j * 3 + 1] = y; nx[j * 3 + 2] = z;
-            bx[j] = x; by[j] = y; bz[j] = z;
-        }
-        __syncthreads();
-    }
-    if (t >= 64) return;
-    {
-        float px[UB], py[UB], pz[UB], md[UB];
-#pragma unroll
-        for (int i = 0; i < UB; ++i) {
-            const int k = t + brev_small<UB>(i) * 64;
-            px[i] = bx[k]; py[i] = by[k]; pz[i] = bz[k];
-            md[i] = 1e10f;
-        }
-        if (t == 0) spick2[0] = 0;
-        float x1 = bx[0], y1 = by[0], z1 = bz[0];
-        for (int j = 1; j < m2; ++j) {
-            float best = -1.f;
-            int bslot = 0;
-#pragma unroll
-            for (int i = 0; i < UB; ++i) {
-                const float dx = px[i] - x1, dy = py[i] - y1, dz = pz[i] - z1;
-                const float d = dist2<FM>(dx, dy, dz);
-                const float d2 = bare_min_f32(d, md[i]);
-                md[i] = d2;
-                const bool gt = d2 > best;
-                bslot = gt ? i : bslot;
-                best = gt ? d2 : best;
-            }
-            const int k = UB == 1 ? t : t + brev_small<UB>(bslot) * 64;
-            float wval; int wk; unsigned wrank;
-            wave_argmax(best, k, bsB, log2bsB, wval, wk, wrank);
-            const int old = wk;
-            x1 = bx[old]; y1 = by[old]; z1 = bz[old];
-            if (t == 0) spick2[j] = old;
-        }
-        __builtin_amdgcn_fence(__ATOMIC_RELEASE, "wavefront");
-        __builtin_amdgcn_wave_barrier();
-        __builtin_amdgcn_fence(__ATOMIC_ACQUIRE, "wavefront");
-        int *idx = idx2_all + (size_t)blockIdx.x * m2;
-        float *nx = nx2_all + (size_t)blockIdx.x * m2 * 3;
-        for (int j = t; j < m2; j += 64) {
-            const int k = spick2[j];
-            idx[j] = k;
-            nx[j * 3 + 0] = bx[k]; nx[j * 3 + 1] = by[k]; nx[j * 3 + 2] = bz[k];
-        }
-    }
+    fps_pair_body<UA, UB, FM>(smem_raw, m2, xyz_all, idx1_all, nx1_all, idx2_all, nx2_all, blockIdx.x);
 }
 
 template <int FM>
@@ -423,7 +295,7 @@
     G4D_REQUIRE(b >= 0 && g4d_fps_gather_pair_supported(n, m1, m2), "g4d_fps_gather_pair_f32: unsupported shape (n=%d m1=%d m2=%d)", n, m1, m2);
     if (b == 0) return G4D_OK;
     G4D_REQUIRE(xyz && idx1 && new_xyz1 && idx2 && new_xyz2, "g4d_fps_gather_pair_f32: null pointer");
-    const size_t lds = 2 * 16 * 16 + (size_t)n * 12 + (size_t)m1 * 16 + (size_t)m2 * 4;
+    const size_t lds = fps_pair_lds_bytes(n, m1, m2);
     hipStream_t s = reinterpret_cast<hipStream_t>(stream);
     G4D_WITH_FM(distance_contraction(), hipLaunchKernelGGL((fps_reg_pair_kernel<4, 4, FM>), dim3(b), dim3(256), lds, s, m2, xyz, idx1, new_xyz1, idx2, new_xyz2))
     return check_launch("g4d_fps_gather_pair_f32");
diff --git a/garment4d_amd/csrc/fps_pair_body.h b/garment4d_amd/csrc/fps_pair_body.h
--- /dev/null
+++ b/garment4d_amd/csrc/fps_pair_body.h
@@ -0,0 +1,142 @@
+#pragma once
+#include "g4d_common.h"
+
+namespace g4d {
+
+template <int U>
+__device__ __host__ constexpr int brev_small(int v) {
+    int r = 0;
+    for (int bit = 1, rb = U >> 1; bit < U; bit <<= 1, rb >>= 1)
+        if (v & bit) r |= rb;
+    return r;
+}
+
+__device__ __forceinline__ void wave_argmax(float best, int k, int bs, int log2bs, float &wval, int &wk, unsigned &wrank) {
+    wval = wave_max_f32(best);
+    const unsigned long long hit = __builtin_amdgcn_ballot_w64(best == wval);
+    int lane;
+    if (__builtin_popcountll(hit) == 1) {
+        lane = __builtin_ctzll(hit);
+        wk = __builtin_amdgcn_readlane(k, lane);
+        wrank = fps_rank(wk, bs, log2bs);
+    } else {
+        const unsigned r = (best == wval) ? fps_rank(k, bs, log2bs) : 0xffffffffu;
+        wrank = wave_min_u32(r);
+        lane = __builtin_ctzll(__builtin_amdgcn_ballot_w64(r == wrank));
+        wk = __builtin_amdgcn_readlane(k, lane);
+    }
+}
+
+__host__ __device__ constexpr size_t fps_pair_lds_bytes(int n, int m1, int m2) { return 2 * 16 * 16 + (size_t)n * 12 + (size_t)m1 * 16 + (size_t)m2 * 4; }
+template <int UA, int UB, int FM>
+__device__ __forceinline__ void fps_pair_body(unsigned char *smem_raw, int m2, const float *__restrict__ xyz_all, int *__restrict__ idx1_all,
+                                              float *__restrict__ nx1_all, int *__restrict__ idx2_all, float *__restrict__ nx2_all, int cloud) {
+    constexpr int T = 256, W = 4, nA = T * UA, bsA = nA, m1 = 64 * UB, bsB = m1;
+    constexpr int log2bsA = UA == 1 ? 8 : (UA == 2 ? 9 : 10), log2bsB = UB == 1 ? 6 : (UB == 2 ? 7 : (UB == 4 ? 8 : 9));
+    float *sx = reinterpret_cast<float *>(smem_raw + 2 * 16 * 16);
+    float *sy = sx + nA;
+    float *sz = sy + nA;
+    int *spick = reinterpret_cast<int *>(sz + nA);
+    float *bx = reinterpret_cast<float *>(spick + m1);
+    float *by = bx + m1;
+    float *bz = by + m1;
+    int *spick2 = reinterpret_cast<int *>(bz + m1);
+    const int t = threadIdx.x;
+    const float *xyz = xyz_all + (size_t)cloud * nA * 3;
+
+    {
+        float px[UA], py[UA], pz[UA], md[UA];
+#pragma unroll
+        for (int i = 0; i < UA; ++i) {
+            const int k = t + brev_small<UA>(i) * T;
+            px[i] = xyz[k * 3 + 0]; py[i] = xyz[k * 3 + 1]; pz[i] = xyz[k * 3 + 2];
+            md[i] = 1e10f;
+            sx[k] = px[i]; sy[k] = py[i]; sz[k] = pz[i];
+        }
+        if (t == 0) spick[0] = 0;
+        __syncthreads();
+        float x1 = sx[0], y1 = sy[0], z1 = sz[0];
+        const int wave = t >> 6;
+        for (int j = 1; j < m1; ++j) {
+            float best = -1.f;
+            int bslot = 0;
+#pragma unroll
+            for (int i = 0; i < UA; ++i) {
+                const float dx = px[i] - x1, dy = py[i] - y1, dz = pz[i] - z1;
+                const float d = dist2<FM>(dx, dy, dz);
+                const float d2 = bare_min_f32(d, md[i]);
+                md[i] = d2;
+                const bool gt = d2 > best;
+                bslot = gt ? i : bslot;
+                best = gt ? d2 : best;
+            }
+            const int k = UA == 1 ? t : t + brev_small<UA>(bslot) * T;
+            float wval; int wk; unsigned wrank;
+            wave_argmax(best, k, bsA, log2bsA, wval, wk, wrank);
+            unsigned long long *buf = reinterpret_cast<unsigned long long *>(smem_raw) + (j & 1) * 16;
+            if ((t & 63) == 0) buf[wave] = ((unsigned long long)__float_as_uint(fmaxf(wval, 0.f)) << 32) | (unsigned)(~wrank);
+            __syncthreads();
+            const unsigned long long key = row_max_u64<W>(buf[t & (W - 1)]);
+            const unsigned rank = ~(unsigned)__builtin_amdgcn_readlane((int)(unsigned)key, W - 1);
+            const unsigned c = __builtin_bitreverse32(rank >> 16) >> (32 - log2bsA);
+            const int old = (int)(((rank & 0xffffu) << log2bsA) | c);
+            x1 = sx[old]; y1 = sy[old]; z1 = sz[old];
+            if (t == 0) spick[j] = old;
+        }
+        __syncthreads();
+        int *idx = idx1_all + (size_t)cloud * m1;
+        float *nx = nx1_all + (size_t)cloud * m1 * 3;
+        for (int j = t; j < m1; j += T) {
+            const int k = spick[j];
+            idx[j] = k;
+            const float x = sx[k], y = sy[k], z = sz[k];
+            nx[j * 3 + 0] = x; nx[j * 3 + 1] = y; nx[j * 3 + 2] = z;
+            bx[j] = x; by[j] = y; bz[j] = z;
+        }
+        __syncthreads();
+    }
+    if (t >= 64) return;
+    {
+        float px[UB], py[UB], pz[UB], md[UB];
+#pragma unroll
+        for (int i = 0; i < UB; ++i) {
+            const int k = t + brev_small<UB>(i) * 64;
+            px[i] = bx[k]; py[i] = by[k]; pz[i] = bz[k];
+            md[i] = 1e10f;
+        }
+        if (t == 0) spick2[0] = 0;
+        float x1 = bx[0], y1 = by[0], z1 = bz[0];
+        for (int j = 1; j < m2; ++j) {
+            float best = -1.f;
+            int bslot = 0;
+#pragma unroll
+            for (int i = 0; i < UB; ++i) {
+                const float dx = px[i] - x1, dy = py[i] - y1, dz = pz[i] - z1;
+                const float d = dist2<FM>(dx, dy, dz);
+                const float d2 = bare_min_f32(d, md[i]);
+                md[i] = d2;
+                const bool gt = d2 > best;
+                bslot = gt ? i : bslot;
+                best = gt ? d2 : best;
+            }
+            const int k = UB == 1 ? t : t + brev_small<UB>(bslot) * 64;
+            float wval; int wk; unsigned wrank;
+            wave_argmax(best, k, bsB, log2bsB, wval, wk, wrank);
+            const int old = wk;
+            x1 = bx[old]; y1 = by[old]; z1 = bz[old];
+            if (t == 0) spick2[j] = old;
+        }
+        __builtin_amdgcn_fence(__ATOMIC_RELEASE, "wavefront");
+        __builtin_amdgcn_wave_barrier();
+        __builtin_amdgcn_fence(__ATOMIC_ACQUIRE, "wavefront");
+        int *idx = idx2_all + (size_t)cloud * m2;
+        float *nx = nx2_all + (size_t)cloud * m2 * 3;
+        for (int j = t; j < m2; j += 64) {
+            const int k = spick2[j];
+            idx[j] = k;
+            nx[j * 3 + 0] = bx[k]; nx[j * 3 + 1] = by[k]; nx[j * 3 + 2] = bz[k];
+        }
+    }
+}
+
+}
diff --git a/garment4d_amd/csrc/index_merge.hip b/garment4d_amd/csrc/index_merge.hip
--- /dev/null
+++ b/garment4d_amd/csrc/index_merge.hip
@@ -0,0 +1,80 @@
+#include "g4d_common.h"
+#include "../../include/g4d_index.h"
+#include "ball_grid_build.h"
+#include "ball_grid_query_body.h"
+#include "fps_pair_body.h"
+
+namespace g4d {
+
+constexpr int kPairN = 1024, kPairM1 = 256;
+
+template <int NS, int FM, bool SET>
+__global__ void __launch_bounds__(256) fps_pair_ball_grid_kernel(int nclouds, int tiles, int n, int m, int qpw, const BgArgs a,
+                                                                const float *__restrict__ new_xyz_all, const float *__restrict__ xyz_all,
+                                                                const unsigned char *__restrict__ ws_all, size_t ws_stride, int cmax, int m2,
+                                                                int *__restrict__ idx1_all, float *__restrict__ nx1_all,
+                                                                int *__restrict__ idx2_all, float *__restrict__ nx2_all) {
+    constexpr size_t kPairBytes = fps_pair_lds_bytes(kPairN, kPairM1, kPairM1), kListBytes = sizeof(int) * 4 * NS * kCap;
+    __shared__ __attribute__((aligned(16))) unsigned char smem[kPairBytes > kListBytes ? kPairBytes : kListBytes];
+    if ((int)blockIdx.x < nclouds) {
+        fps_pair_body<4, 4, FM>(smem, m2, new_xyz_all, idx1_all, nx1_all, idx2_all, nx2_all, (int)blockIdx.x);
+        return;
+    }
+    const int lin = (int)blockIdx.x - nclouds;
+    const int b = lin / tiles;
+    ball_grid_query_body<NS, FM, SET>(reinterpret_cast<int (*)[NS][kCap]>(smem), n, m, qpw, a, new_xyz_all, xyz_all, ws_all, ws_stride, cmax,
+                                      lin - b * tiles, b);
+}
+
+template <int NS, int FM, bool SET>
+static void pair_query_launch(unsigned blocks, hipStream_t st, int b, int tiles, int n, int m, int qpw, const BgArgs &a, const float *new_xyz,
+                              const float *xyz, const void *ws, int m2, int *idx1, float *nx1, int *idx2, float *nx2) {
+    hipLaunchKernelGGL((fps_pair_ball_grid_kernel<NS, FM, SET>), dim3(blocks), dim3(256), 0, st, b, tiles, n, m, qpw, a, new_xyz, xyz,
+                       reinterpret_cast<const unsigned char *>(ws), grid_cloud_bytes(n), grid_cmax(n), m2, idx1, nx1, idx2, nx2);
+}
+
+template <bool SET>
+static int pair_query_entry(const char *name, int b, int n, int m, int nscales, const float *radii, const int *nsamples, const float *new_xyz,
+                            const float *xyz, int *const *idx, const void *grid, float grid_rmax, int m1, int m2, int *idx1, float *new_xyz1,
+                            int *idx2, float *new_xyz2, g4d_stream_t stream) {
+    G4D_REQUIRE(b >= 0 && n >= 1 && nscales >= 1 && nscales <= 4 && b <= 65535, "%s: bad sizes", name);
+    G4D_REQUIRE(g4d_fps_gather_pair_supported(m, m1, m2), "%s: unsupported sampling shape (m=%d m1=%d m2=%d)", name, m, m1, m2);
+    G4D_REQUIRE(radii && nsamples && idx, "%s: null pointer", name);
+    BgArgs a = {};
+    for (int s = 0; s < nscales; ++s) {
+        G4D_REQUIRE(nsamples[s] > 0 && idx[s], "%s: bad scale %d", name, s);
+        G4D_REQUIRE(radii[s] <= grid_rmax, "%s: radius %g exceeds the radius the grid was built for (%g)", name, radii[s], grid_rmax);
+        a.radius2[s] = radii[s] * radii[s];
+        a.nsample[s] = nsamples[s];
+        a.idx[s] = idx[s];
+    }
+    if (b == 0) return G4D_OK;
+    G4D_REQUIRE(new_xyz && xyz && grid && idx1 && new_xyz1 && idx2 && new_xyz2, "%s: null pointer", name);
+    const int qpw = grid_query_qpw((long long)b * m);
+    const int tiles = (m + 4 * qpw - 1) / (4 * qpw);
+    const unsigned blocks = (unsigned)b * (unsigned)(tiles + 1);
+    hipStream_t st = reinterpret_cast<hipStream_t>(stream);
+    G4D_WITH_FM(distance_contraction(), switch (nscales) {
+        case 1: pair_query_launch<1, FM, SET>(blocks, st, b, tiles, n, m, qpw, a, new_xyz, xyz, grid, m2, idx1, new_xyz1, idx2, new_xyz2); break;
+        case 2: pair_query_launch<2, FM, SET>(blocks, st, b, tiles, n, m, qpw, a, new_xyz, xyz, grid, m2, idx1, new_xyz1, idx2, new_xyz2); break;
+        case 3: pair_query_launch<3, FM, SET>(blocks, st, b, tiles, n, m, qpw, a, new_xyz, xyz, grid, m2, idx1, new_xyz1, idx2, new_xyz2); break;
+        default: pair_query_launch<4, FM, SET>(blocks, st, b, tiles, n, m, qpw, a, new_xyz, xyz, grid, m2, idx1, new_xyz1, idx2, new_xyz2); break;
+    })
+    return check_launch(name);
+}
+
+}
+
+extern "C" int g4d_fps_pair_ball_grid_query_set_f32(int b, int n, int m, int nscales, const float *radii, const int *nsamples,
+                                                    const float *new_xyz, const float *xyz, int *const *idx, const void *grid, float grid_rmax,
+                                                    int m1, int m2, int *idx1, float *new_xyz1, int *idx2, float *new_xyz2, g4d_stream_t stream) {
+    return g4d::pair_query_entry<true>("g4d_fps_pair_ball_grid_query_set_f32", b, n, m, nscales, radii, nsamples, new_xyz, xyz, idx, grid, grid_rmax,
+                                       m1, m2, idx1, new_xyz1, idx2, new_xyz2, stream);
+}
+
+extern "C" int g4d_fps_pair_ball_grid_query_f32(int b, int n, int m, int nscales, const float *radii, const int *nsamples, const float *new_xyz,
+                                                const float *xyz, int *const *idx, const void *grid, float grid_rmax, int m1, int m2, int *idx1,
+                                                float *new_xyz1, int *idx2, float *new_xyz2, g4d_stream_t stream) {
+    return g4d::pair_query_entry<false>("g4d_fps_pair_ball_grid_query_f32", b, n, m, nscales, radii, nsamples, new_xyz, xyz, idx, grid, grid_rmax,
+                                        m1, m2, idx1, new_xyz1, idx2, new_xyz2, stream);
+}
diff --git a/garment4d_amd/encoder.py b/garment4d_amd/encoder.py
--- a/garment4d_amd/encoder.py
+++ b/garment4d_amd/encoder.py
@@ -94,7 +94,14 @@
                     pre_nx[0], grid0 = fused.fps_gather_grid(xyz, SAs[0].npoint, max(r0))
                 else:
                     pre_nx[0] = fused.fps_gather(xyz, SAs[0].npoint)
-                pair = fused.fps_gather_pair(pre_nx[0], SAs[1].npoint, SAs[2].npoint)
+                pair = None
+                if grid0 is not None:
+                    merged = fused.fps_pair_ball_query(r0, [g.nsample for g in SAs[0].groupers], xyz, pre_nx[0], grid0, SAs[1].npoint, SAs[2].npoint,
+                                                       set_form=SAs[0].pool_method == "max_pool" and _T().bq_set)
+                    if merged is not None:
+                        pair, pre_idx[0] = merged[:2], merged[2]
+                if pair is None:
+                    pair = fused.fps_gather_pair(pre_nx[0], SAs[1].npoint, SAs[2].npoint)
                 if pair is not None:
                     pre_nx[1], pre_nx[2] = pair
                 else:
diff --git a/garment4d_amd/fused.py b/garment4d_amd/fused.py
--- a/garment4d_amd/fused.py
+++ b/garment4d_amd/fused.py
@@ -422,6 +422,23 @@
     n1, n2 = torch.empty((B, m1, 3), dtype=torch.float32, device=dev), torch.empty((B, m2, 3), dtype=torch.float32, device=dev)
     _lib.call("g4d_fps_gather_pair_f32", B, N, m1, m2, xyz.data_ptr(), i1.data_ptr(), n1.data_ptr(), i2.data_ptr(), n2.data_ptr(), _lib.stream_ptr())
     return n1, n2
+
+
+def fps_pair_ball_query(radii, nsamples, xyz, new_xyz, grid, m1, m2, set_form=False):
+    B, N, _ = _chk(xyz).shape
+    P = _chk(new_xyz).shape[1]
+    if not (_T().pair_in_ball_query and _T().fps_pair and 0 < B <= 65535 and N > 0 and 1 <= len(radii) <= 4 and grid
+            and _lib.lib().g4d_fps_gather_pair_supported(P, m1, m2)):
+        return None
+    _lib.index_lib()
+    dev = xyz.device
+    outs = [torch.empty((B, P, ns), dtype=torch.int32, device=dev) for ns in nsamples]
+    i1, i2 = torch.empty((B, m1), dtype=torch.int32, device=dev), torch.empty((B, m2), dtype=torch.int32, device=dev)
+    n1, n2 = torch.empty((B, m1, 3), dtype=torch.float32, device=dev), torch.empty((B, m2, 3), dtype=torch.float32, device=dev)
+    _lib.call("g4d_fps_pair_ball_grid_query_set_f32" if set_form else "g4d_fps_pair_ball_grid_query_f32", B, N, P, len(radii), _floats(radii),
+              _ints(nsamples), new_xyz.data_ptr(), xyz.data_ptr(), _ptrs(outs), grid[0].data_ptr(), grid[1], m1, m2, i1.data_ptr(), n1.data_ptr(),
+              i2.data_ptr(), n2.data_ptr(), _lib.stream_ptr())
+    return n1, n2, outs
 
 
 
diff --git a/garment4d_amd/tuning.py b/garment4d_amd/tuning.py
--- a/garment4d_amd/tuning.py
+++ b/garment4d_amd/tuning.py
@@ -31,6 +31,7 @@
     grid_min_n: int = 4096
     bq_set: bool = True
     fps_pair: bool = True
+    pair_in_ball_query: bool = True
     bq_multi: bool = True
     search_multi: bool = True
     three_nn_grid_min_m: int = 4096
@@ -87,7 +88,8 @@
         use_wave=_env_flag("G4D_MLP_WAVE", d.use_wave), use_chain=_env_flag("G4D_MLP_CHAIN", d.use_chain), stream_gemm=_env_flag("G4D_GEMM_STREAM", d.stream_gemm),
         bf16_min_rows=_env_int("G4D_BF16_MIN_ROWS", d.bf16_min_rows), overlap_sampling=_env_flag("G4D_OVERLAP_SAMPLING", d.overlap_sampling),
         lanes_sort=_env_flag("G4D_BQ_LANES_SORT", d.lanes_sort), coherent_lanes=_env_flag("G4D_BQ_LANES", d.coherent_lanes),
-        grid_min_n=_env_int("G4D_BQ_GRID_MIN_N", d.grid_min_n), bq_set=_env_flag("G4D_BQ_SET", d.bq_set), fps_pair=_env_flag("G4D_FPS_PAIR", d.fps_pair), bq_multi=_env_flag("G4D_BQ_MULTI", d.bq_multi),
+        grid_min_n=_env_int("G4D_BQ_GRID_MIN_N", d.grid_min_n), bq_set=_env_flag("G4D_BQ_SET", d.bq_set), fps_pair=_env_flag("G4D_FPS_PAIR", d.fps_pair),
+        pair_in_ball_query=_env_flag("G4D_PAIR_IN_BQ", d.pair_in_ball_query), bq_multi=_env_flag("G4D_BQ_MULTI", d.bq_multi),
         search_multi=_env_flag("G4D_SEARCH_MULTI", d.search_multi), three_nn_grid_min_m=_env_int("G4D_NN_GRID_MIN_M", d.three_nn_grid_min_m),
         nn_cells=_env_flag("G4D_NN_CELLS", d.nn_cells), nn_multi=_env_flag("G4D_NN_MULTI", d.nn_multi), nn_prune=_env_flag("G4D_NN_PRUNE", d.nn_prune), sa_xyz_pair=_env_flag("G4D_SA_XYZ_PAIR", d.sa_xyz_pair),
         use_sa_xyz=_env_flag("G4D_SA_XYZ", d.use_sa_xyz), sa_xyz_table=_env_flag("G4D_SA_XYZ_TABLE", d.sa_xyz_table), sa_table=_env_flag("G4D_SA_TABLE", d.sa_table),
diff --git a/include/g4d_index.h b/include/g4d_index.h
--- /dev/null
+++ b/include/g4d_index.h
@@ -0,0 +1,21 @@
+#ifndef G4D_INDEX_H
+#define G4D_INDEX_H
+
+#include "g4d.h"
+
+#ifdef __cplusplus
+extern "C" {
+#endif
+
+int g4d_fps_pair_ball_grid_query_set_f32(int b, int n, int m, int nscales, const float *radii, const int *nsamples, const float *new_xyz,
+                                         const float *xyz, int *const *idx, const void *grid, float grid_rmax, int m1, int m2, int *idx1,
+                                         float *new_xyz1, int *idx2, float *new_xyz2, g4d_stream_t stream);
+
+int g4d_fps_pair_ball_grid_query_f32(int b, int n, int m, int nscales, const float *radii, const int *nsamples, const float *new_xyz,
+                                     const float *xyz, int *const *idx, const void *grid, float grid_rmax, int m1, int m2, int *idx1,
+                                     float *new_xyz1, int *idx2, float *new_xyz2, g4d_stream_t stream);
+
+#ifdef __cplusplus
+}
+#endif
+#endif
```

Result: no change. 55100 (median of 6 runs) (+1.9%).
